# crowsonkb/style_transfer

Measured on AMD Instinct MI355X. Metric: tile-iterations/sec, VGG-19 2048px/1024-tile (fwd+bwd, Gram/content losses, regularizers, Adam step), higher is better.
Workload: dtype f32 (fp16x2-split MFMA, fp32 accumulate)

## Files before the change

include/stx.h:

```cpp
#ifndef STX_H_
#define STX_H_

#include <stddef.h>
#include <stdint.h>

#ifdef __cplusplus
extern "C" {
#endif

typedef struct stx_engine stx_engine;

typedef enum stx_status {
    STX_OK = 0,
    STX_ERR_ARG = -1,
    STX_ERR_HIP = -2,
    STX_ERR_STATE = -3,
    STX_ERR_UNSUPPORTED = -4,
    STX_ERR_NOMEM = -5
} stx_status;

typedef enum stx_mem { STX_HOST = 0, STX_DEVICE = 1 } stx_mem;

typedef enum stx_layer_type {
    STX_LAYER_INPUT = 0, STX_LAYER_CONV = 1, STX_LAYER_RELU = 2, STX_LAYER_POOL = 3
} stx_layer_type;

typedef enum stx_pool_mode { STX_POOL_MAX = 0, STX_POOL_AVE = 1 } stx_pool_mode;

typedef struct stx_layer_desc {
    const char *name;
    int type;
    const char *bottom;
    const char *top;
    int num_output;
    int kernel_size;
    int pad;
    int stride;
    int pool_mode;
} stx_layer_desc;

const char *stx_version(void);
const char *stx_last_error(void);
int stx_reread_env(void);
int stx_device_count(int *count);
int stx_device_name(int device, char *buf, size_t buf_len);

int stx_engine_create(int device, const stx_layer_desc *layers, int n_layers, stx_engine **out);
int stx_engine_create_shared(stx_engine *primary, stx_engine **out);
void stx_engine_destroy(stx_engine *e);
int stx_set_conv_weights(stx_engine *e, const char *conv_layer, const float *weights,
                         const float *bias, int mem);
int stx_sync(stx_engine *e);
int stx_fence(stx_engine *e, unsigned long long *ticket);
int stx_fence_wait(stx_engine *e, unsigned long long ticket);
int stx_engine_wait(stx_engine *e, stx_engine *other);
typedef enum stx_query {
    STX_Q_SHARED_ENGINES = 0,
    STX_Q_TARGET_UPLOADS = 1,
    STX_Q_TARGET_BYTES = 2,
    STX_Q_WEIGHT_BYTES = 3,
    STX_Q_TILE_EVALS = 4,
    STX_Q_PEERS_WITHOUT_ACCESS = 5
} stx_query;
int stx_engine_query(stx_engine *e, int what, double *value);
int stx_engine_device(stx_engine *e, int *device);
int stx_engine_stream(stx_engine *e, void **hip_stream);

int stx_malloc(stx_engine *e, size_t bytes, void **dev_ptr);
int stx_free(stx_engine *e, void *dev_ptr);
int stx_memset_async(stx_engine *e, void *dev_ptr, int value, size_t bytes);
int stx_memcpy_async(stx_engine *e, void *dst, int dst_mem, const void *src, int src_mem,
                     size_t bytes);

typedef struct stx_content_target {
    int content_index;
    const char *layer;
    int channels, height, width;
    const float *features;
    int mem;
} stx_content_target;

typedef struct stx_style_target {
    int style_index;
    const char *layer;
    int channels;
    const float *gram;
    int mem;
} stx_style_target;

int stx_set_contents_and_styles(stx_engine *e, const stx_content_target *contents, int n_contents,
                                const stx_style_target *styles, int n_styles);

typedef struct stx_style_mask {
    int style_index;
    int H, W;
    const float *mask;
    int mem;
} stx_style_mask;
int stx_set_style_masks(stx_engine *e, const stx_style_mask *masks, int n);

typedef struct stx_stat_target {
    const char *layer;
    int channels;
    const float *mean;
    const float *sd;
    int mem;
    double weight;
} stx_stat_target;
int stx_set_stat_targets(stx_engine *e, const stx_stat_target *targets, int n);

int stx_features_tile(stx_engine *e, const float *img, int img_mem, int th, int tw,
                      const char *const *layers, int n_layers, float *const *out, int out_mem);

typedef struct stx_tap {
    const char *layer;
    double layer_weight;
    int is_content;
    double content_weight;
    int is_style;
    double style_weight;
    int is_dd;
    double dd_weight;
} stx_tap;

int stx_sc_grad_tile(stx_engine *e, const float *img, int img_mem, int th, int tw,
                     const int roll_xy[2], const int start_yx[2], const stx_tap *taps, int n_taps,
                     double *loss_out, float *grad_out, int grad_mem, int sync_now);

int stx_tile_buffers(stx_engine *e, int th, int tw, float **tile_in, float **grad_out);

int stx_gram_matrix(stx_engine *e, const float *feat, int feat_mem, int channels, int hw,
                    float *gram_out, int gram_mem);

int stx_feature_stats(stx_engine *e, const float *feat, int feat_mem, int channels, int hw,
                      float *mean_out, float *sd_out, int out_mem);


int stx_image_cut_tile(stx_engine *e, const float *img, int H, int W, const int roll_xy[2],
                       int y0, int x0, int th, int tw, float *tile);
int stx_image_put_tile(stx_engine *e, float *grad, int H, int W, const int roll_xy[2],
                       int y0, int x0, int th, int tw, const float *tile_grad);

int stx_image_mask_map(stx_engine *e, const float *mask, int H, int W, int scale, float *out);
int stx_map_place(stx_engine *e, float *dst, int channels, int dst_h, int dst_w, int y0, int x0,
                  const float *src, int h, int w);
int stx_map_roll_add(stx_engine *e, float *acc, const float *src, int channels, int h, int w,
                     const int roll_xy[2], double alpha, double init_divisor);

int stx_image_resample(stx_engine *e, const float *src, int channels, int H, int W, float *dst,
                       int out_h, int out_w, const int *bounds_x, const double *weights_x,
                       int ksize_x, const int *bounds_y, const double *weights_y, int ksize_y,
                       int clamp_min_zero);

int stx_image_regularizers(stx_engine *e, const float *img, float *grad, int H, int W,
                           const float mean_bgr[3], double tv_scale, double tv_power,
                           double p_scale, double p_power, const float *aux, double aux_scale,
                           const int aux_roll_xy[2], double *loss_out);

int stx_image_swt_haar(stx_engine *e, const float *img, float *grad, int H, int W,
                       const int roll_xy[2], double scale, double power, double *loss_out);

int stx_image_swt_haar_levels(stx_engine *e, const float *img, float *grad, int H, int W, int levels,
                              const int roll_xy[2], double scale, double power, double *loss_out);

int stx_image_swt_daub_levels(stx_engine *e, const float *img, float *grad, int H, int W,
                              int order, int levels, const int *roll_xy,
                              double scale, double power, double *loss_out);

int stx_adam_step(stx_engine *e, float *params, const float *grad, float *g1, float *g2, float *p1,
                  float *avg_out, size_t n, double lr, double b1, double b2, double bp1,
                  double corr1, double corr2, double corrp);

int stx_vec_dot(stx_engine *e, const float *x, const float *y, size_t n, double *out_host_sync);
int stx_vec_axpy(stx_engine *e, double a, const float *x, float *y, size_t n);
int stx_vec_scale(stx_engine *e, double a, float *x, size_t n);
int stx_vec_mean_abs(stx_engine *e, const float *x, size_t n, double *out_host_sync);
int stx_vec_dot_async(stx_engine *e, const float *x, const float *y, size_t n, double *out_dev);
int stx_vec_abs_sum_async(stx_engine *e, const float *x, size_t n, double *out_dev);
int stx_vec_axpy_dev(stx_engine *e, double c1, const double *a_dev, double da, double c2,
                     const double *b_dev, double db, const float *x, float *y, size_t n);
int stx_vec_scale_dev(stx_engine *e, double c, const double *den_dev, double den_div, float *x,
                      size_t n);
int stx_vec_axpy_dot_dev(stx_engine *e, double c1, const double *a_dev, double da, double c2,
                         const double *b_dev, double db, double scale_c, const double *scale_den_dev,
                         double scale_div, const float *x, const float *src, float *y, const float *z,
                         size_t n, double *out_dev);
int stx_vec_lbfgs_pair(stx_engine *e, const float *g_new, float *g_old, const float *s, float *y, size_t n,
                       double *out_dev2, double *sy_host_sync);
int stx_vec_scale2_axpy(stx_engine *e, double c1, double c2, float *s, float *params, size_t n);

int stx_image_step_stats(stx_engine *e, const float *avg, float *old, int H, int W,
                         double stats[2]);
int stx_image_step_stats_async(stx_engine *e, const float *avg, float *old, int H, int W,
                               double raw_sums[2]);

int stx_image_to_u8(stx_engine *e, const float *img, int H, int W, const float mean_bgr[3],
                    uint8_t *out_rgb_u8);

int stx_image_to_u8_luma(stx_engine *e, const float *img, const float *content, int H, int W,
                         const float mean_bgr[3], uint8_t *out_rgb_u8);
int stx_image_color_stats(stx_engine *e, const float *img, int H, int W, double out_host_sync[9]);
int stx_image_color_affine(stx_engine *e, const float *src, float *dst, int H, int W, const double A[9],
                           const double b[3], const float mean_bgr[3]);

size_t stx_image_lap_floats(int H, int W, int n_pools, const int *pools);
int stx_image_lap_target(stx_engine *e, const float *content, int H, int W, int n_pools,
                         const int *pools, float *target_out);
int stx_image_lap(stx_engine *e, const float *img, float *grad, int H, int W, int n_pools,
                  const int *pools, const double *weights, const float *target, double scale,
                  double *loss_out);

int stx_op_conv_forward(stx_engine *e, const float *x, int Cin, int H, int W, const float *w,
                        const float *b, int Cout, int ksize, int relu, float *y);
int stx_op_conv_backward_data(stx_engine *e, const float *dy, int Cout, int H, int W,
                              const float *w, int Cin, int ksize, const float *relu_mask_data,
                              float *dx);
int stx_op_pool_forward(stx_engine *e, const float *x, int C, int H, int W, int mode, float *y);
int stx_op_pool_backward(stx_engine *e, const float *dy, const float *x, int C, int H, int W,
                         int mode, const float *relu_mask_data, float *dx);

int stx_op_style_terms(stx_engine *e, const float *feat, int channels, int h, int w,
                       const float *gram_target, float *s_out, float *normalized_out,
                       double *half_sumsq, double *abs_sum);
int stx_op_masked_style_terms(stx_engine *e, const float *feat, int channels, int h, int w,
                              const float *mask_map, int mh, int mw, int oy, int ox, const int roll_xy[2],
                              const float *gram_target, float *sgrad_out, double out[3]);
int stx_op_stat_terms(stx_engine *e, const float *feat, int channels, int h, int w, const float *MU,
                      const float *SD, float *s_out, double out[2]);
int stx_op_content_terms(stx_engine *e, const float *feat, int channels, int h, int w,
                         const float *content, int content_h, int content_w, int oy, int ox,
                         const int roll_xy[2], float *normalized_out, double sums[2]);

int stx_profile_enable(stx_engine *e, int on);
int stx_profile_read(stx_engine *e, char *buf, size_t buf_len, size_t *needed);

int stx_last_tile_ms(stx_engine *e, float *ms);

int stx_last_tile_flops(stx_engine *e, double *algorithmic, double *issued);

int stx_clock_marks(stx_engine *e, int on);
int stx_clock_marks_read(stx_engine *e, double *mhz, int max_values, int *n_values);

#ifdef __cplusplus
}
#endif
#endif
```

style_transfer_amd/csrc/common.h:

```cpp
#pragma once

#include <hip/hip_runtime.h>

#include <vector>

#include <cstdarg>
#include <cstdio>
#include <functional>
#include <string>

#include "stx.h"

namespace stx {

constexpr float kEps = 1.1920928955078125e-07f;

void set_error(const char *fmt, ...);

const char *sw_env(const char *name);
void sw_reread();

#define STX_HIP(call)                                                                       \
    do {                                                                                    \
        hipError_t err__ = (call);                                                          \
// ... 40 lines not shown
#pragma unroll
    for (int k = 0; k < NV; ++k) {
        const float s = wave_sum_f(v[k]);
        if ((threadIdx.x & 63) == 0) red[k][threadIdx.x >> 6] = s;
    }
    __syncthreads();
    if (threadIdx.x == 0) {
#pragma unroll
        for (int k = 0; k < NV; ++k)
            partials[k * gridDim.x + blockIdx.x] = red[k][0] + red[k][1] + red[k][2] + red[k][3];
    }
}

__device__ __forceinline__ unsigned pool_max_code(float v00, float v01, float v10, float v11, bool hx,
                                                  bool hy) {
    unsigned arg = 0;
    float best = v00;
    if (hx && v01 > best) best = v01, arg = 1;
    if (hy && v10 > best) best = v10, arg = 2;
    if (hx && hy && v11 > best) best = v11, arg = 3;
    return arg | (best > 0.f ? 4u : 0u);
}
__device__ __forceinline__ unsigned pool_ave_code(float v00, float v01, float v10, float v11, bool hx,
                                                  bool hy) {
    return (v00 > 0.f ? 1u : 0u) | (hx && v01 > 0.f ? 2u : 0u) | (hy && v10 > 0.f ? 4u : 0u) |
           (hx && hy && v11 > 0.f ? 8u : 0u);
}
#endif


enum ConvEpilogue {
    kEpiForward = 0,
    kEpiDgrad = 1,
    kEpiSymm = 2,
    kEpiDgradInject = 3,
    kEpiPartial = 4
};

struct ContentWindow {
    int C, fh, fw;
    int ch, cw;
    int oy, ox;
    int sy, sx;
};

struct ConvInject {
    const float *sgrad = nullptr, *s_abs_sum = nullptr;
    float s_coef = 0.f;
    const float *content = nullptr, *c_sums = nullptr, *feat = nullptr;
    float c_coef = 0.f;
    ContentWindow win{};
};

struct ConvProblem {
    const float *x;
    const float *w;
    float *y;
    const float *bias;
    const float *mask;
    float *partials;
    int K, M, H, W;
    int ksize;
    int relu;
    int epilogue;
    ConvInject inject;
    unsigned char *pool_codes = nullptr;
    unsigned char *in_codes = nullptr;
    const unsigned char *mask_codes = nullptr;
    unsigned char *out_codes = nullptr;
    bool wants_codes = false;
    bool skip_y = false;
    float *pool_out = nullptr;
    int pool_mode = 0;
    float *splitk_ws = nullptr;
    size_t splitk_ws_floats = 0;
    long long *clock_out = nullptr;
    const unsigned *x_amax = nullptr;
    unsigned *y_amax = nullptr;
    const unsigned char *pin_codes = nullptr;
    int pin_mode = 0;
    bool pin_mask = false;
#ifdef STX_EXPERIMENT_BF3
    const void *x_split = nullptr;
#endif
};

enum class ConvFamily { Direct, Wino2, H2 };

struct ConvConfig {
    ConvFamily family;
    int id;
    int bm;
    int kc;
    int pr, pc;
    int threads;
    size_t lds_bytes;
};

ConvConfig conv_pick_config(int ksize, int K, int M, int H, int W);
ConvConfig conv_config_by_id(int id);
bool direct_takes_inject(const ConvConfig &cfg);
int conv_num_workgroups(const ConvConfig &cfg, int M, int H, int W);
size_t conv_packed_floats(const ConvConfig &cfg, int K, int M, int ksize);
int conv_pack_weights(hipStream_t s, const float *w_caffe, int Mo, int Ko, int ksize,
                      int transpose_flip, const ConvConfig &cfg, float *packed);
int conv_launch(hipStream_t s, const ConvConfig &cfg, const ConvProblem &p, bool packed_weights);
int direct_splitk_factor(const ConvConfig &cfg, const ConvProblem &p, bool packed_weights);

int splitk_reduce_launch(hipStream_t s, const ConvProblem &p, int ksplit);
int splitk_reduce_items_launch(hipStream_t s, const ConvProblem &p, const ConvConfig &cfg, int slices,
                               int item_base, int items);
__host__ __device__ inline void wino2_item_tiles(int lt, int m_tiles, int n_patches, int &pt, int &mt) {
    pt = lt / m_tiles;
    mt = lt - pt * m_tiles;
    if (m_tiles == 8 && (n_patches & 7) == 0) {
        const int g = lt >> 5, r = lt & 31;
        mt = (g & 1) * 4 + (r & 3);
        pt = (g >> 1) * 8 + (r >> 2);
    }
}

struct WinoArgs {
    const float *x;
    const float *w;
    float *y;
    const float *bias;
    const float *mask;
    int K, M, H, W;
    int n_chunks, tiles_x, tiles_y, m_tiles, ksplit;
    int w_tile_stride;
    int x_bytes, w_bytes;
    int relu;
    ConvInject inj;
    float *pool_out;
    int pool_mode;
    unsigned char *pool_codes;
    int skip_y = 0;
    unsigned char *out_codes = nullptr;
    unsigned char *in_codes = nullptr;
    const unsigned char *mask_codes = nullptr;
    long long *clock_out = nullptr;
    int item_base = 0;
    const unsigned *x_amax = nullptr;
    unsigned *y_amax = nullptr;
    const unsigned char *pin_codes = nullptr;
    int pin_mode = 0, pin_mask = 0;
#ifdef STX_EXPERIMENT_BF3
    int vp_rows = 0, vp_tp = 0;
#endif
};

bool conv_first_usable(int K, int M, int ksize);
int conv_first_workgroups(int H, int W);
int conv_first_launch(hipStream_t s, const float *x, const float *w_caffe, const float *bias, float *y,
                      int K, int H, int W, int relu, float *gram_partials, unsigned *y_amax = nullptr);

ConvConfig wino2_config(int geometry = 0);
int wino2_pick_geometry(int H, int W);
size_t wino2_packed_floats(int K, int M);
int wino2_pack_weights(hipStream_t s, const float *w_caffe, int Mo, int Ko, int transpose_flip,
                       float *packed);
int wino2_launch(hipStream_t s, const ConvConfig &cfg, const ConvProblem &p, int ksplit);
bool wino2_fuses_pool(const ConvProblem &p);
bool wino2_uses_relu_codes(const ConvProblem &p, int ksplit);
bool wino2_writes_out_codes(const ConvConfig &cfg, const ConvProblem &p);
int wino2_splitk_factor(const ConvConfig &cfg, const ConvProblem &p);
struct Wino2Tail { int items, slices; };
Wino2Tail wino2_tail_split(const ConvConfig &cfg, const ConvProblem &p);
int wino2_max_slices(const ConvConfig &cfg, const ConvProblem &p);

constexpr int kAmaxSlots = 64;
ConvConfig h2_config(int mb, int pb = 1);
ConvConfig h2_pick_config(const ConvProblem &p);
bool h2_usable(const ConvProblem &p);
size_t h2_packed_floats(int K, int M);
int h2_pack_weights(hipStream_t s, const float *w_caffe, int Mo, int Ko, int transpose_flip, float *packed);
int h2_launch(hipStream_t s, const ConvConfig &cfg, const ConvProblem &p, int ksplit);
int h2_splitk_factor(const ConvConfig &cfg, const ConvProblem &p);
bool h2_fuses_pool(const ConvProblem &p);
bool h2_takes_pooled_input(const ConvConfig &cfg, const ConvProblem &p);
int absmax_launch(hipStream_t s, const float *x, size_t n, unsigned *slots);

size_t conv_small_packed_floats(int K);
int conv_small_pack(hipStream_t s, const float *w_caffe, int Mo, int Ko, int transpose_flip,
                    float *packed);
int conv_small_launch(hipStream_t s, const float *x, const float *packed, float *y,
                      const float *mask, int K, int M, int H, int W);

bool conv_h2_enabled();
struct ConvTuner { int device; hipStream_t stream; hipEvent_t ev0, ev1; std::function<int(const ConvConfig &, const float **)> bank; };
int conv_choose(const ConvProblem &p, bool winograd, const ConvTuner *tuner, ConvConfig *out);
struct ConvBank { int key; size_t floats; std::function<int(hipStream_t, const float *w_caffe, float *packed)> pack; };
ConvBank conv_bank(const ConvConfig &cfg, int dir, int Mo, int Ko, int ksize);
ConvBank conv_small_bank(int Mo, int Ko);
int conv_dispatch(hipStream_t s, const ConvConfig &cfg, const ConvProblem &p, double *flop_algorithmic,
                  double *flop_issued);
int conv_splitk_factor(const ConvConfig &cfg, const ConvProblem &p);
size_t conv_splitk_floats(const ConvConfig &cfg, const ConvProblem &p);
bool conv_takes_clock(const ConvConfig &cfg);
bool conv_fuses_pool(const ConvConfig &cfg, const ConvProblem &p);
bool conv_writes_pool_codes(const ConvConfig &cfg);
bool conv_reads_x_amax(const ConvConfig &cfg);
bool conv_leaves_y_amax(const ConvConfig &cfg);
bool conv_takes_inject(const ConvConfig &cfg);
bool conv_takes_pooled_input(const ConvConfig &cfg, const ConvProblem &p);
bool conv_uses_relu_codes(const ConvConfig &cfg, const ConvProblem &p, int ksplit);
bool conv_writes_out_codes(const ConvConfig &cfg, const ConvProblem &p, int ksplit);

int pool_forward_launch(hipStream_t s, const float *x, int C, int H, int W, int mode, float *y,
                        unsigned char *codes = nullptr);
int pool_backward_codes_launch(hipStream_t s, const float *dy, const unsigned char *codes, int C,
                               int H, int W, int mode, bool relu_mask, float *dx);
int pool_backward_launch(hipStream_t s, const float *dy, const float *x, int C, int H, int W,
                         int mode, bool relu_mask, float *dx);

struct GramPlan {
    int C, HW, splits, tiles;
    int parts;
    size_t partial_floats;
};
GramPlan gram_plan(int C, int HW);
bool gram_h2_usable(const float *feat, int C, int HW);
int gram_partials_launch(hipStream_t s, const float *feat, const GramPlan &plan, float *partials,
                         const unsigned *f_amax = nullptr);
int gram_finish_blocks(const GramPlan &plan);
int gram_finish_launch(hipStream_t s, const float *partials, const GramPlan &plan, float *gram_out,
                       const float *target, float *dsym, float *sumsq, unsigned short *pieces = nullptr,
                       const unsigned *f_amax = nullptr, float *block_out = nullptr);

size_t symm_pieces_elems(int C);
int symm_num_workgroups(int C, int HW);
bool symm_bf3_usable(const float *feat, const float *out, int C, int HW);
bool symm_h2_usable(const float *feat, const float *out, int C, int HW);
int symm_h2_launch(hipStream_t s, const float *feat, const float *dsym, const unsigned *d_amax, int n_damax,
                   const unsigned *f_amax, float *out, float *partials, int C, int HW);
int symm_bf3_launch(hipStream_t s, const float *feat, const float *dsym, unsigned short *pieces,
                    bool pieces_ready, float *out, float *partials, int C, int HW);

#ifdef __HIPCC__
__device__ __forceinline__ int content_origin_y(const ContentWindow &w) { return w.oy - w.sy; }
__device__ __forceinline__ int content_origin_x(const ContentWindow &w) { return w.ox - w.sx; }
__device__ __forceinline__ size_t content_index(const ContentWindow &w, int c, int y, int x) {
    int yy = (content_origin_y(w) + y) % w.ch;
    int xx = (content_origin_x(w) + x) % w.cw;
    if (yy < 0) yy += w.ch;
    if (xx < 0) xx += w.cw;
    return ((size_t)c * w.ch + yy) * w.cw + xx;
}
#endif

struct SumJob {
    const float *src;
    int n;
    float *dst;
};
int sum_jobs_launch(hipStream_t s, const SumJob *jobs, int n_jobs);
int content_sums_launch(hipStream_t s, const float *feat, const float *content,
                        const ContentWindow &win, float *sums , std::vector<SumJob> *defer = nullptr);
int inject_style_launch(hipStream_t s, float *diff, const float *sgrad, size_t n,
                        const float *abs_sum, float coef, bool accumulate, unsigned *y_amax = nullptr);
int inject_content_launch(hipStream_t s, float *diff, const float *feat, const float *content,
                          const ContentWindow &win, const float *sums, float coef, bool accumulate,
                          unsigned *y_amax = nullptr);
int relu_inplace_launch(hipStream_t s, float *x, size_t n);
int sum_partials_launch(hipStream_t s, const float *partials, int n, float *out);
int sum_partials2_launch(hipStream_t s, const float *a, int na, float *out_a, const float *b, int nb,
                         float *out_b);

constexpr int kMaskParts = 1024;
constexpr int kMaskSgradParts = 2048;
int mask_map_launch(hipStream_t s, const float *mask, int H, int W, int scale, float *out);
int mask_apply_launch(hipStream_t s, const float *feat, const float *map, const ContentWindow &win, float *fm,
                      float *m2_partials, int *n_parts);
int mask_target_launch(hipStream_t s, const float *gs, int C, const float *m2_partials, int n_parts, int HW,
                       float *out, float *a_out);
int mask_sgrad_launch(hipStream_t s, float *sgrad, const float *map, const ContentWindow &win, const float *a,
                      float *partials, int *n_parts);

constexpr int kStatSlice = 16384;
constexpr float kStatEps = 1e-5f;
int stat_slices(int HW);
size_t stat_scratch_floats(int C, int HW);
int stat_partials_launch(hipStream_t s, const float *feat, int C, int HW, float *partials);
int stat_finish_launch(hipStream_t s, const float *partials, int C, int HW, const float *MU, const float *SD,
                       float *table, float *e_out, float *mean_out, float *sd_out);
int stat_grad_launch(hipStream_t s, const float *feat, int C, int HW, const float *table, float *sgrad,
                     float *abs_partials, int *n_parts);

int cut_tile_launch(hipStream_t s, const float *img, int H, int W, int rx, int ry, int y0, int x0,
                    int th, int tw, float *tile);
int put_tile_launch(hipStream_t s, float *grad, int H, int W, int rx, int ry, int y0, int x0,
                    int th, int tw, const float *tile);
int place_window_launch(hipStream_t s, float *dst, int dh, int dw, int y0, int x0, const float *src,
                        int C, int h, int w);
int roll_add_launch(hipStream_t s, float *acc, const float *src, int C, int h, int w, int sx, int sy,
                    float alpha, bool init);
int resample_launch(hipStream_t s, int axis, const float *src, int C, int H, int W, float *dst,
                    int OH, int OW, const int *bounds, const double *k, int ksize, int clamp);
int finish_partials_launch(hipStream_t s, const float *partials, int n, double *out_dev);
int finish_partials_n_launch(hipStream_t s, const float *partials, int n, int nv, double *out_dev);
int regularizers_launch(hipStream_t s, const float *img, float *grad, int H, int W,
                        const float mean[3], float tv_scale, float tv_power, float p_scale,
                        float p_power, const float *aux, float aux_scale, int aux_rx, int aux_ry,
                        double *loss_terms , float *scratch, size_t scratch_floats);

int swt_padded_side(int H, int W);
int swt_haar_launch(hipStream_t s, const float *img, float *grad, int H, int W, int rx, int ry,
                    float scale, float power, double *loss_term, float *scratch,
                    size_t scratch_floats);
void swt_levels_scratch(int H, int W, size_t *tmp_floats, size_t *partial_floats);
int swt_haar_levels_launch(hipStream_t s, const float *img, float *grad, int H, int W, int levels,
                           int rx, int ry, float scale, float power, double *loss_term, float *tmp,
                           float *partials);
void swt_daub_table(int order, int levels, int N, std::vector<float> *taps, int *hl);
int swt_table_launch(hipStream_t s, const float *img, float *grad, int H, int W, const float *table,
                     int ntaps, int hl, int rx, int ry, float scale, float power,
                     double *loss_term, float *tmp, float *partials);

constexpr int kLapMaxPools = 4;
struct LapLevels {
    int n;
    int lp[kLapMaxPools], hp[kLapMaxPools], wp[kLapMaxPools], off[kLapMaxPools];
};
size_t lap_levels(int H, int W, int n_pools, const int *pools, LapLevels *lv);
size_t lap_scratch_floats(size_t map_floats);
int lap_target_launch(hipStream_t s, const float *content, int H, int W, const LapLevels &lv,
                      float *target, float *scratch);
int lap_launch(hipStream_t s, const float *img, float *grad, int H, int W, const LapLevels &lv,
               size_t map_floats, const float *coefs, const float *target, double *loss_terms,
               float *scratch);

int adam_launch(hipStream_t s, float *params, const float *grad, float *g1, float *g2, float *p1,
                float *avg, size_t n, double lr, double b1, double b2, double bp1, double c1,
                double c2, double cp);
int dot_launch(hipStream_t s, const float *x, const float *y, size_t n, double *out_dev,
               float *scratch, size_t scratch_floats);
int abs_sum_launch(hipStream_t s, const float *x, size_t n, double *out_dev, float *scratch,
                   size_t scratch_floats);
int axpy_launch(hipStream_t s, float a, const float *x, float *y, size_t n);
int scale_launch(hipStream_t s, float a, float *x, size_t n);
// ... 22 lines not shown
```

style_transfer_amd/csrc/conv_first.hip:

```cpp

#include <algorithm>
#include <cstdlib>

#include "bf16x3.h"
#include "common.h"

namespace stx {

namespace {

constexpr int kFP = 128;
constexpr int kFM = 64;
constexpr int kPW = kFP + 4;
constexpr int kPatch = 12 * kPW;
constexpr int kFLd = kFP + 4;
constexpr int kTile = kFM * kFLd;
constexpr int kNT = 256;
constexpr int kPL = (9 * (kFP + 2) + kNT - 1) / kNT;

typedef float f32x16 __attribute__((ext_vector_type(16)));
typedef float f32x4 __attribute__((ext_vector_type(4)));
typedef unsigned int u32x4f __attribute__((ext_vector_type(4)));

__device__ __forceinline__ int sgpr(int v) { return __builtin_amdgcn_readfirstlane(v); }
__device__ __forceinline__ void lds_barrier() { asm volatile("s_waitcnt lgkmcnt(0)\n\ts_barrier" ::: "memory"); }

struct FirstArgs {
    const float *x;
    const float *w;
    const float *bias;
    float *y;
    float *gram;
    unsigned *y_amax;
    int K, H, W, tiles_x, n_tiles, relu, vec_store, strided;
};

}

template <bool GRAM, int STORE>
__global__ __launch_bounds__(kNT, GRAM ? 2 : 3) void conv_first_kernel(FirstArgs a) {
    constexpr int kWork = 2 * kPatch + kTile;
    static_assert(kFM * kFM <= kWork, "the Gram tile must fit the working set");
    __shared__ __attribute__((aligned(16))) float lds[kWork];
    float *const patch = lds;
    float *const tile = lds + 2 * kPatch;
    const int tid = threadIdx.x, lane = tid & 63;
    const int wave = __builtin_amdgcn_readfirstlane(tid >> 6);
    const int l31 = lane & 31, half = lane >> 5;
    const size_t HW = (size_t)a.H * a.W;

    float aw[2][18];
#pragma unroll
    for (int s = 0; s < 18; ++s) {
        const int c = 2 * (s / 9) + half, tap = s % 9;
#pragma unroll
        for (int mb = 0; mb < 2; ++mb)
            aw[mb][s] = c < a.K ? a.w[((size_t)(mb * 32 + l31) * a.K + c) * 9 + tap] : 0.f;
    }
#pragma unroll
    for (int s = 0; s < 18; ++s) asm volatile("" ::"v"(aw[0][s]), "v"(aw[1][s]));
    float bias_r[2];
#pragma unroll
    for (int mb = 0; mb < 2; ++mb) bias_r[mb] = a.bias ? a.bias[mb * 32 + l31] : 0.f;
    asm volatile("" ::"v"(bias_r[0]), "v"(bias_r[1]));

    const __amdgpu_buffer_rsrc_t rx = __builtin_amdgcn_make_buffer_rsrc(
        const_cast<float *>(a.x), 0, (int)((size_t)a.K * HW * 4), 0x00020000);
    constexpr unsigned kOob = 0x80000000u;
    int p_row[kPL], p_col[kPL], p_off[kPL];
#pragma unroll
    for (int n = 0; n < kPL; ++n) {
        const int e = tid + n * kNT;
        const int pr = e / (kFP + 2), col = e - pr * (kFP + 2);
        const int c = pr / 3, r = pr - 3 * c;
        const bool live = e < 9 * (kFP + 2) && c < a.K;
        p_row[n] = live ? r - 1 : -(1 << 28);
        p_col[n] = col - 1;
        p_off[n] = (c * a.H + r - 1) * a.W + col - 1;
    }
    auto patch_load = [&](int t, float (&preg)[kPL]) {
        const int ty = sgpr(t < 0 ? -4 : t / a.tiles_x);
        const int x0 = sgpr(t < 0 ? 0 : (t - ty * a.tiles_x) * kFP);
        const int origin = sgpr(ty * a.W + x0);
#pragma unroll
        for (int n = 0; n < kPL; ++n) {
            const bool ok = (unsigned)(ty + p_row[n]) < (unsigned)a.H && (unsigned)(x0 + p_col[n]) < (unsigned)a.W;
            const unsigned off = ok ? (unsigned)(origin + p_off[n]) * 4u : kOob;
            preg[n] = __builtin_bit_cast(float, __builtin_amdgcn_raw_buffer_load_b32(rx, off, 0, 0));
        }
    };
    int p_dst[kPL];
#pragma unroll
    for (int n = 0; n < kPL; ++n) {
        const int e = tid + n * kNT;
        const int pr = e / (kFP + 2), col = e - pr * (kFP + 2);
        p_dst[n] = e < 9 * (kFP + 2) ? pr * kPW + col : -1;
    }
    auto patch_store = [&](int buf, const float (&preg)[kPL]) {
#pragma unroll
        for (int n = 0; n < kPL; ++n)
            if (p_dst[n] >= 0) patch[buf * kPatch + p_dst[n]] = preg[n];
    };

    f32x16 g[3];
    if (GRAM) {
#pragma unroll
        for (int b = 0; b < 3; ++b)
#pragma unroll
            for (int r = 0; r < 16; ++r) g[b][r] = 0.f;
    }

    const int per_wg = a.strided ? 1 : (a.n_tiles + (int)gridDim.x - 1) / (int)gridDim.x;
    const int grid = a.strided ? (int)gridDim.x : 1;
    const int t_begin = a.strided ? (int)blockIdx.x : (int)blockIdx.x * per_wg;
    const int t_end = a.strided ? a.n_tiles : (t_begin + per_wg < a.n_tiles ? t_begin + per_wg : a.n_tiles);
    const __amdgpu_buffer_rsrc_t ry = __builtin_amdgcn_make_buffer_rsrc(
        a.y, 0, STORE == 2 ? 0 : (int)(unsigned)((size_t)kFM * HW * 4), 0x00020000);
    constexpr unsigned kOobY = 0xfffffff0u;
    const int y_ch0 = tid >> 5, y_c4 = (tid & 31) * 4;
    const unsigned y_voff = (unsigned)(((size_t)y_ch0 * HW + y_c4) * 4);
    const bool track = a.y_amax != nullptr;
    float amax = 0.f;
    auto segment = [&](int t, int buf, const float (&pin)[kPL], float (&pout)[kPL]) {
        patch_load(t + 2 * grid < t_end ? t + 2 * grid : -1, pout);
        const int ty = sgpr(t / a.tiles_x), x0 = sgpr((t - ty * a.tiles_x) * kFP);

        f32x16 acc[2];
#pragma unroll
        for (int mb = 0; mb < 2; ++mb)
#pragma unroll
            for (int r = 0; r < 16; ++r) acc[mb][r] = 0.f;
        const float *pb = patch + buf * kPatch + half * (3 * kPW) + wave * 32 + l31;
#pragma unroll
        for (int s = 0; s < 18; ++s) {
            const int q = s / 9, ky = (s % 9) / 3, kx = s % 3;
            const float xv = pb[(2 * q * 3 + ky) * kPW + kx];
            acc[0] = __builtin_amdgcn_mfma_f32_32x32x2f32(xv, aw[0][s], acc[0], 0, 0, 0);
            acc[1] = __builtin_amdgcn_mfma_f32_32x32x2f32(xv, aw[1][s], acc[1], 0, 0, 0);
        }
        const bool ragged = x0 + kFP > a.W;
        const int room = a.W - x0 - wave * 32 - 4 * half;
#pragma unroll
        for (int mb = 0; mb < 2; ++mb)
#pragma unroll
            for (int j = 0; j < 4; ++j) {
                f32x4 v = {acc[mb][4 * j], acc[mb][4 * j + 1], acc[mb][4 * j + 2], acc[mb][4 * j + 3]};
                v += bias_r[mb];
                if (a.relu) {
                    v.x = fmaxf(v.x, 0.f), v.y = fmaxf(v.y, 0.f);
                    v.z = fmaxf(v.z, 0.f), v.w = fmaxf(v.w, 0.f);
                }
                if (ragged) {
                    v.x = 8 * j + 0 < room ? v.x : 0.f, v.y = 8 * j + 1 < room ? v.y : 0.f;
                    v.z = 8 * j + 2 < room ? v.z : 0.f, v.w = 8 * j + 3 < room ? v.w : 0.f;
                }
                if (track) amax = fmaxf(fmaxf(amax, fmaxf(fabsf(v.x), fabsf(v.y))), fmaxf(fabsf(v.z), fabsf(v.w)));
                *reinterpret_cast<f32x4 *>(tile + (mb * 32 + l31) * kFLd + wave * 32 + 8 * j + 4 * half) = v;
            }
        lds_barrier();

        {
            float *const yrow = a.y + (size_t)ty * a.W + x0;
            const unsigned origin = (unsigned)sgpr((ty * a.W + x0) * 4);
            const unsigned vo4 = x0 + y_c4 < a.W ? y_voff : kOobY;
#pragma unroll
            for (int n = 0; n < kFM * (kFP / 4) / kNT; ++n) {
                const f32x4 v = *reinterpret_cast<const f32x4 *>(tile + (y_ch0 + 8 * n) * kFLd + y_c4);
                if (STORE == 2) {
                    float *const dst = yrow + (size_t)(y_ch0 + 8 * n) * HW + y_c4;
                    if (x0 + y_c4 + 0 < a.W) dst[0] = v.x;
                    if (x0 + y_c4 + 1 < a.W) dst[1] = v.y;
                    if (x0 + y_c4 + 2 < a.W) dst[2] = v.z;
                    if (x0 + y_c4 + 3 < a.W) dst[3] = v.w;
                    continue;
                }
                const unsigned so = origin + (unsigned)sgpr((int)((unsigned)(8 * n) * (unsigned)HW * 4u));
                if (STORE == 0) {
                    __builtin_amdgcn_raw_buffer_store_b128(__builtin_bit_cast(u32x4f, v), ry, vo4, so, 0);
                } else {
                    const float vs[4] = {v.x, v.y, v.z, v.w};
#pragma unroll
                    for (int i = 0; i < 4; ++i)
                        __builtin_amdgcn_raw_buffer_store_b32(__builtin_bit_cast(unsigned, vs[i]), ry,
                                                              x0 + y_c4 + i < a.W ? y_voff + 4u * i : kOobY, so, 0);
                }
            }
        }
        if (GRAM) {
#pragma unroll
            for (int st = 0; st < 2; ++st) {
                bf16x8 p[2][3];
#pragma unroll
                for (int mb = 0; mb < 2; ++mb) {
                    const float *q = tile + (mb * 32 + l31) * kFLd + wave * 32 + st * 16 + half * 8;
                    const f32x4 lo = *reinterpret_cast<const f32x4 *>(q);
                    const f32x4 hi = *reinterpret_cast<const f32x4 *>(q + 4);
                    const float xv[8] = {lo.x, lo.y, lo.z, lo.w, hi.x, hi.y, hi.z, hi.w};
                    split3_bf16(xv, p[mb][0], p[mb][1], p[mb][2]);
                }
                g[0] = mfma_split6(p[0], p[0], g[0]);
                g[1] = mfma_split6(p[1], p[0], g[1]);
                g[2] = mfma_split6(p[1], p[1], g[2]);
            }
        }
        if (t + grid < t_end) patch_store(buf ^ 1, pin);
        lds_barrier();
    };

    for (int i = tid; i < 2 * kPatch; i += kNT) patch[i] = 0.f;
    lds_barrier();
    float pa[kPL], pb2[kPL];
    const int t0 = t_begin;
    if (t0 < t_end) {
        patch_load(t0, pa);
        patch_store(0, pa);
    }
    if (t0 + grid < t_end) patch_load(t0 + grid, pa);
    lds_barrier();
    for (int t = t0; t < t_end; t += 2 * grid) {
        segment(t, 0, pa, pb2);
        if (t + grid < t_end) segment(t + grid, 1, pb2, pa);
    }

    if (track) {
#pragma unroll
        for (int d = 32; d >= 1; d >>= 1) amax = fmaxf(amax, __shfl_xor(amax, d));
        lds_barrier();
        if (lane == 0) lds[wave] = amax;
        lds_barrier();
        if (tid == 0)
            atomicMax(a.y_amax + (blockIdx.x & (kAmaxSlots - 1)),
                      __builtin_bit_cast(unsigned, fmaxf(fmaxf(lds[0], lds[1]), fmaxf(lds[2], lds[3]))));
    }
    if (GRAM) {
        lds_barrier();
        float *const red = lds;
#pragma unroll 1
        for (int w = 0; w < 4; ++w) {
            if (wave == w) {
#pragma unroll
                for (int r = 0; r < 16; ++r) {
                    const int row = (r & 3) + 8 * (r >> 2) + 4 * half;
                    float *q0 = red + row * kFM + l31, *q1 = red + (32 + row) * kFM + l31;
                    q0[0] = w == 0 ? g[0][r] : q0[0] + g[0][r];
                    if (w == 0) q0[32] = 0.f;
                    q1[0] = w == 0 ? g[1][r] : q1[0] + g[1][r];
                    q1[32] = w == 0 ? g[2][r] : q1[32] + g[2][r];
                }
            }
            lds_barrier();
        }
        float *out = a.gram + (size_t)blockIdx.x * (kFM * kFM);
#pragma unroll
        for (int n = 0; n < 4; ++n) {
            const int e = tid + kNT * n;
            reinterpret_cast<float4 *>(out)[e] = reinterpret_cast<const float4 *>(red)[e];
        }
    }
}

bool conv_first_usable(int K, int M, int ksize) {
    const char *env = sw_env("STX_CONV_FIRST_FUSED");
    if (env && atoi(env) == 0) return false;
    return ksize == 3 && K >= 1 && K <= 3 && M == kFM;
}

int conv_first_workgroups(int H, int W) {
    const long tiles = (long)H * ceil_div(W, kFP);
    return (int)std::min<long>(tiles, 512);
}
static int conv_first_plain_workgroups(int H, int W) {
    const long tiles = (long)H * ceil_div(W, kFP);
    const char *env = sw_env("STX_FIRST_WGS");
    return (int)std::min<long>(tiles, env ? atoi(env) : 768);
}

int conv_first_launch(hipStream_t s, const float *x, const float *w_caffe, const float *bias, float *y,
                      int K, int H, int W, int relu, float *gram_partials, unsigned *y_amax) {
    if (4.0 * K * (double)H * W >= 2147483648.0) {
        set_error("conv_first_launch: a %d x %d plane is beyond the buffer-addressing limit", H, W);
        return STX_ERR_UNSUPPORTED;
    }
    FirstArgs a;
    a.x = x;
    a.w = w_caffe;
    a.bias = bias;
    a.y = y;
    a.gram = gram_partials;
    a.y_amax = y_amax;
    a.K = K;
    a.H = H;
    a.W = W;
    a.tiles_x = ceil_div(W, kFP);
    a.n_tiles = H * a.tiles_x;
    a.relu = relu;
    a.vec_store = W % 4 == 0 && (reinterpret_cast<uintptr_t>(y) & 15) == 0;
    const int grid = gram_partials ? conv_first_workgroups(H, W) : conv_first_plain_workgroups(H, W);
    {
        const char *env = sw_env("STX_FIRST_STRIDED");
        a.strided = env && atoi(env) != 0;
    }
    const int store = 4.0 * kFM * (double)H * W >= 4294967280.0 ? 2 : a.vec_store ? 0 : 1;
#define STX_FIRST(G, S) conv_first_kernel<G, S><<<grid, kNT, 0, s>>>(a)
    if (gram_partials) {
        if (store == 0) STX_FIRST(true, 0);
        else if (store == 1) STX_FIRST(true, 1);
        else STX_FIRST(true, 2);
    } else {
        if (store == 0) STX_FIRST(false, 0);
        else if (store == 1) STX_FIRST(false, 1);
        else STX_FIRST(false, 2);
    }
#undef STX_FIRST
    STX_CHECK_LAUNCH();
    return STX_OK;
}

}
```

style_transfer_amd/csrc/conv_mfma.hip:

```cpp

#include <algorithm>
#include <cstdlib>

#include "common.h"

namespace stx {

typedef float f32x16 __attribute__((ext_vector_type(16)));
typedef unsigned int u32x4 __attribute__((ext_vector_type(4)));

struct ConvKernelArgs {
    const float *x;
    const float *w;
    float *y;
    const float *bias;
    const float *mask;
    float *partials;
    int K, M, H, W;
    int n_chunks;
    int tiles_x, tiles_y;
    int m_tiles;
    int ksplit;
    int w_row_stride;
    int w_tile_stride;
// ... 522 lines not shown
    if (p.epilogue == kEpiForward && packed) return launch_variant<ID, kEpiForward, true>(s, cfg, a, n_wg);
    if constexpr (v.inject) {
        if (inject && packed) return launch_variant<ID, kEpiDgradInject, true>(s, cfg, a, n_wg);
    }
    if (p.epilogue == kEpiDgrad && packed && !inject) return launch_variant<ID, kEpiDgrad, true>(s, cfg, a, n_wg);
    set_error("conv_launch: no kernel for config %d epilogue %d packed %d", cfg.id, p.epilogue, (int)packed);
    return STX_ERR_UNSUPPORTED;
}

int conv_launch(hipStream_t s, const ConvConfig &cfg, const ConvProblem &p, bool packed) {
    const ConvVariant &v = kVariants[cfg.id];
    if (v.ks != p.ksize) {
        set_error("conv_launch: config %d is %dx%d, problem is %dx%d", cfg.id, v.ks, v.ks, p.ksize,
                  p.ksize);
        return STX_ERR_ARG;
    }
    ConvKernelArgs a;
    a.x = p.x;
    a.w = p.w;
    a.y = p.y;
    a.bias = p.bias;
    a.mask = p.mask;
    a.partials = p.partials;
    a.K = p.K;
    a.M = p.M;
    a.H = p.H;
    a.W = p.W;
    a.n_chunks = ceil_div(p.K, cfg.kc);
    a.tiles_x = ceil_div(p.W, cfg.pc);
    a.tiles_y = ceil_div(p.H, cfg.pr);
    a.m_tiles = ceil_div(p.M, cfg.bm);
    a.w_row_stride = packed ? cfg.bm : p.M;
    a.w_tile_stride = packed ? a.n_chunks * cfg.kc * p.ksize * p.ksize * cfg.bm : 0;
    const double xb = 4.0 * p.K * (double)p.H * p.W;
    const double wb = packed ? 4.0 * (double)conv_packed_floats(cfg, p.K, p.M, p.ksize)
                             : 4.0 * (double)p.K * p.M;
    if (xb >= 2147483648.0 || wb >= 2147483648.0) {
        set_error("conv_launch: a %d x %d x %d plane set exceeds the 2 GiB buffer-addressing limit "
                  "of the kernel (use a smaller --tile-size)", p.K, p.H, p.W);
        return STX_ERR_UNSUPPORTED;
    }
    a.x_bytes = (int)xb;
    a.w_bytes = (int)wb;
    a.relu = p.relu;
    a.inj = p.inject;
    a.ksplit = 1;
    const bool inject = p.epilogue == kEpiDgrad && (p.inject.sgrad || p.inject.content);
    int n_wg = conv_num_workgroups(cfg, p.M, p.H, p.W);
    const int ksplit = direct_splitk_factor(cfg, p, packed);
    const bool split = ksplit > 1 && p.splitk_ws &&
                       p.splitk_ws_floats >= (size_t)ksplit * p.M * p.H * p.W;
    if (split) {
        a.ksplit = ksplit;
        a.y = p.splitk_ws;
        n_wg *= ksplit;
    }

    switch (cfg.id) {
#define STX_DISPATCH(ID) \
    case ID: return dispatch_variant<ID>(s, cfg, p, a, n_wg, packed, inject, split ? ksplit : 1);
        STX_DISPATCH(0)
        STX_DISPATCH(1)
        STX_DISPATCH(2)
        STX_DISPATCH(3)
        STX_DISPATCH(4)
        STX_DISPATCH(8)
        STX_DISPATCH(9)
        STX_DISPATCH(10)
        STX_DISPATCH(11)
        STX_DISPATCH(5)
        STX_DISPATCH(6)
        STX_DISPATCH(7)
        STX_DISPATCH(12)
        STX_DISPATCH(13)
        STX_DISPATCH(14)
#undef STX_DISPATCH
    }
    set_error("conv_launch: no kernel for config %d epilogue %d packed %d", cfg.id, p.epilogue, (int)packed);
    return STX_ERR_UNSUPPORTED;
}

static SplitReduceArgs splitk_reduce_args(const ConvProblem &p, int ksplit) {
    SplitReduceArgs r;
    r.part = p.splitk_ws;
    r.y = p.y;
    r.bias = p.bias;
    r.mask = p.mask;
    r.inj = p.inject;
    r.ksplit = ksplit;
    r.M = p.M;
    r.HW = p.H * p.W;
    r.W = p.W;
    r.relu = p.relu;
    r.epilogue = p.epilogue;
    r.y_amax = p.y_amax;
    return r;
}

int splitk_reduce_launch(hipStream_t s, const ConvProblem &p, int ksplit) {
    const SplitReduceArgs r = splitk_reduce_args(p, ksplit);
    const size_t n = (size_t)p.M * p.H * p.W;
    if (n >= ((size_t)1 << 32)) {
        set_error("splitk_reduce: %zu elements", n);
        return STX_ERR_UNSUPPORTED;
    }
    const uintptr_t ptrs = reinterpret_cast<uintptr_t>(r.part) | reinterpret_cast<uintptr_t>(r.y) |
                           reinterpret_cast<uintptr_t>(r.mask) | reinterpret_cast<uintptr_t>(r.inj.feat) |
                           reinterpret_cast<uintptr_t>(r.inj.sgrad);
    const char *env = sw_env("STX_REDUCE_VEC");
    if ((p.H * p.W) % 4 == 0 && (ptrs & 15) == 0 && n < (1u << 31) && !(env && atoi(env) == 0)) {
        const size_t n4 = n / 4;
        splitk_reduce_vec4_kernel<<<(int)std::min<size_t>((n4 + 255) / 256, p.y_amax ? 1024 : 4096), 256, 0, s>>>(r);
        STX_CHECK_LAUNCH();
        return STX_OK;
    }
    splitk_reduce_kernel<<<(int)std::min<size_t>((n + 255) / 256, p.y_amax ? 1024 : 4096), 256, 0, s>>>(r);
    STX_CHECK_LAUNCH();
    return STX_OK;
}

int splitk_reduce_items_launch(hipStream_t s, const ConvProblem &p, const ConvConfig &cfg, int slices,
                               int item_base, int items) {
    const SplitReduceArgs r = splitk_reduce_args(p, slices);
    if ((size_t)p.M * p.H * p.W >= ((size_t)1 << 32)) {
        set_error("splitk_reduce: %zu elements", (size_t)p.M * p.H * p.W);
        return STX_ERR_UNSUPPORTED;
    }
    ItemRange range;
    range.item_base = item_base;
    range.m_tiles = ceil_div(p.M, 64);
    range.tiles_x = ceil_div(p.W, cfg.pc);
    range.tiles_y = ceil_div(p.H, cfg.pr);
    range.pr = cfg.pr;
    range.pc = cfg.pc;
    range.H = p.H;
    splitk_reduce_items_kernel<<<items * kItemBlocks, 256, 0, s>>>(r, range);
    STX_CHECK_LAUNCH();
    return STX_OK;
}

}

namespace stx {

typedef float f32x4 __attribute__((ext_vector_type(4)));

struct SmallConvArgs {
    const float *x;
    const float *w;
    float *y;
    const float *mask;
    int K, M, H, W, n_chunks, tiles_x, x_bytes, w_bytes;
    int n_wg, wg_per_xcd;
};

template <int KC, int PR, bool VEC>
__global__ __launch_bounds__(256) void conv3x3_m4_kernel(SmallConvArgs a) {
    constexpr int PC = 64, XR = PR + 2, XC = VEC ? PC + 8 : PC + 2, X0 = VEC ? 3 : 0, NT = 256, RW = PR / 4;
    constexpr int X_FLOATS = KC * XR * XC, W_FLOATS = KC * 9 * 4;
    constexpr int NX = (KC * XR * (PC + 2) + NT - 1) / NT;
    constexpr int NV = KC * XR * (PC / 4);
    constexpr int NVT = (NV + NT - 1) / NT;
    constexpr int NH = KC * XR * 2;
    static_assert(W_FLOATS / 4 <= NT, "one float4 of weights per thread");
    constexpr int NHT = (NH + NT - 1) / NT;
    __shared__ __attribute__((aligned(16))) float Xl[X_FLOATS];
    __shared__ __attribute__((aligned(16))) float Wl[W_FLOATS];
    const int tid = threadIdx.x, lane = tid & 63;
    const int wave = __builtin_amdgcn_readfirstlane(tid >> 6);
    const int patch = sgpr((int)(blockIdx.x & 7) * a.wg_per_xcd + (int)(blockIdx.x >> 3));
    if (patch >= a.n_wg) return;
    const int y0 = sgpr((patch / a.tiles_x) * PR), x0 = sgpr((patch % a.tiles_x) * PC);
    const int HW = a.H * a.W;
    constexpr unsigned kOob = 0x80000000u;
    const bool big = a.x_bytes == 0;
    __amdgpu_buffer_rsrc_t rx = __builtin_amdgcn_make_buffer_rsrc(
        const_cast<float *>(a.x), 0, a.x_bytes, 0x00020000);
    const __amdgpu_buffer_rsrc_t rw = __builtin_amdgcn_make_buffer_rsrc(
        const_cast<float *>(a.w), 0, a.w_bytes, 0x00020000);
    unsigned xvoff[VEC ? 1 : NX], vvoff[VEC ? NVT : 1], hvoff[NHT];
    int vdst[VEC ? NVT : 1], hdst[NHT];
    if (VEC) {
#pragma unroll
        for (int n = 0; n < NVT; ++n) {
            const int e = tid + n * NT;
            const int ci = e / (XR * (PC / 4)), rem = e - ci * (XR * (PC / 4));
            const int r = rem / (PC / 4), c4 = rem - r * (PC / 4);
            const int yy = y0 - 1 + r, xx = x0 + 4 * c4;
            const bool ok = e < NV && (unsigned)yy < (unsigned)a.H && xx < a.W;
            vvoff[n] = ok ? (unsigned)(ci * HW + yy * a.W + xx) * 4u : kOob;
            vdst[n] = e < NV ? (ci * XR + r) * XC + X0 + 1 + 4 * c4 : -1;
        }
#pragma unroll
        for (int n = 0; n < NHT; ++n) {
            const int e = tid + n * NT;
            const int ci = e / (XR * 2), rem = e - ci * (XR * 2);
            const int r = rem >> 1, side = rem & 1;
            const int yy = y0 - 1 + r, xx = side ? x0 + PC : x0 - 1;
            const bool ok = e < NH && (unsigned)yy < (unsigned)a.H && (unsigned)xx < (unsigned)a.W;
            hvoff[n] = ok ? (unsigned)(ci * HW + yy * a.W + xx) * 4u : kOob;
            hdst[n] = e < NH ? (ci * XR + r) * XC + X0 + (side ? PC + 1 : 0) : -1;
        }
    } else {
#pragma unroll
        for (int n = 0; n < NX; ++n) {
            const int e = tid + n * NT;
            const int ci = e / (XR * XC), rem = e - ci * (XR * XC);
            const int r = rem / XC, c = rem - r * XC;
            const int yy = y0 - 1 + r, xx = x0 - 1 + c;
            const bool ok = e < X_FLOATS && (unsigned)yy < (unsigned)a.H && (unsigned)xx < (unsigned)a.W;
            xvoff[n] = ok ? (unsigned)(ci * HW + yy * a.W + xx) * 4u : kOob;
        }
    }
    const unsigned wvoff = tid < W_FLOATS / 4 ? (unsigned)tid * 16u : kOob;
    unsigned xreg[VEC ? 1 : NX], hreg[NHT];
    u32x4 vreg[VEC ? NVT : 1];
    u32x4 wreg;
    auto load_stage = [&](int chunk) {
        wreg = __builtin_amdgcn_raw_buffer_load_b128(rw, wvoff, (unsigned)chunk * (W_FLOATS * 4u), 0);
        unsigned xs = (unsigned)sgpr((int)((unsigned)chunk * (unsigned)(KC * HW) * 4u));
        if (big) {
            const int k0 = sgpr(chunk * KC);
            const int nk = a.K - k0 < KC ? a.K - k0 : KC;
            rx = __builtin_amdgcn_make_buffer_rsrc(const_cast<float *>(a.x) + (size_t)k0 * (size_t)HW, 0,
                                                   (nk > 0 ? nk : 0) * HW * 4, 0x00020000);
            xs = 0;
        }
        if (VEC) {
#pragma unroll
            for (int n = 0; n < NVT; ++n) vreg[n] = __builtin_amdgcn_raw_buffer_load_b128(rx, vvoff[n], xs, 0);
#pragma unroll
            for (int n = 0; n < NHT; ++n) hreg[n] = __builtin_amdgcn_raw_buffer_load_b32(rx, hvoff[n], xs, 0);
        } else {
#pragma unroll
            for (int n = 0; n < NX; ++n) xreg[n] = __builtin_amdgcn_raw_buffer_load_b32(rx, xvoff[n], xs, 0);
        }
    };
    auto store_stage = [&]() {
        if (tid < W_FLOATS / 4) reinterpret_cast<u32x4 *>(Wl)[tid] = wreg;
        if (VEC) {
#pragma unroll
            for (int n = 0; n < NVT; ++n)
                if (vdst[n] >= 0) *reinterpret_cast<u32x4 *>(Xl + vdst[n]) = vreg[n];
#pragma unroll
            for (int n = 0; n < NHT; ++n)
                if (hdst[n] >= 0) reinterpret_cast<unsigned *>(Xl)[hdst[n]] = hreg[n];
        } else {
#pragma unroll
            for (int n = 0; n < NX; ++n) {
                const int e = tid + n * NT;
                if (e < X_FLOATS) reinterpret_cast<unsigned *>(Xl)[e] = xreg[n];
            }
        }
    };
    f32x4 acc[RW];
#pragma unroll
    for (int r = 0; r < RW; ++r) acc[r] = f32x4{0.f, 0.f, 0.f, 0.f};
    const float *wl = Wl + (lane & 3);
    const float *xl = Xl + (wave * RW) * XC + X0 + lane;

    load_stage(0);
    store_stage();
    __syncthreads();
    for (int chunk = 0; chunk < a.n_chunks; ++chunk) {
        const bool more = chunk + 1 < a.n_chunks;
        if (more) load_stage(chunk + 1);
#pragma unroll
        for (int ci = 0; ci < KC; ++ci) {
#pragma unroll
            for (int t = 0; t < 9; ++t) {
                const float av = wl[(ci * 9 + t) * 4];
#pragma unroll
                for (int r = 0; r < RW; ++r) {
                    const float bv = xl[ci * (XR * XC) + (r + t / 3) * XC + t % 3];
                    acc[r] = __builtin_amdgcn_mfma_f32_4x4x1f32(av, bv, acc[r], 0, 0, 0);
                }
            }
        }
        __syncthreads();
        if (more) {
            store_stage();
            __syncthreads();
        }
    }
    const int xx = x0 + lane;
#pragma unroll
    for (int r = 0; r < RW; ++r) {
        const int yy = y0 + wave * RW + r;
        if (yy < a.H && xx < a.W) {
#pragma unroll
            for (int m = 0; m < 4; ++m) {
                if (m < a.M) {
                    const size_t idx = (size_t)m * HW + (size_t)yy * a.W + xx;
                    float v = acc[r][m];
                    if (a.mask) v = a.mask[idx] > 0.f ? v : 0.f;
                    a.y[idx] = v;
                }
            }
        }
    }
}

constexpr int kSmallKC = 4, kSmallPR = 16;

size_t conv_small_packed_floats(int K) { return (size_t)ceil_div(K, kSmallKC) * kSmallKC * 9 * 4; }

__global__ void pack_small_kernel(const float *__restrict__ w, int Mo, int Ko, int transpose_flip,
                                  int M, int K, int kpad, float *__restrict__ packed) {
    const int total = kpad * 9 * 4;
    for (int i = blockIdx.x * blockDim.x + threadIdx.x; i < total; i += gridDim.x * blockDim.x) {
        const int m = i & 3, t = (i >> 2) % 9, k = i / 36;
        float v = 0.f;
        if (m < M && k < K)
            v = transpose_flip ? w[((size_t)k * Ko + m) * 9 + (8 - t)] : w[((size_t)m * Ko + k) * 9 + t];
        packed[i] = v;
    }
}

int conv_small_pack(hipStream_t s, const float *w_caffe, int Mo, int Ko, int transpose_flip,
                    float *packed) {
    const int M = transpose_flip ? Ko : Mo, K = transpose_flip ? Mo : Ko;
    const int kpad = ceil_div(K, kSmallKC) * kSmallKC;
    pack_small_kernel<<<ceil_div(kpad * 36, 256), 256, 0, s>>>(w_caffe, Mo, Ko, transpose_flip, M, K,
                                                               kpad, packed);
    STX_CHECK_LAUNCH();
    return STX_OK;
}

int conv_small_launch(hipStream_t s, const float *x, const float *packed, float *y,
                      const float *mask, int K, int M, int H, int W) {
    if (M > 4) {
        set_error("conv_small_launch: M = %d > 4", M);
        return STX_ERR_ARG;
    }
    const double xb = 4.0 * K * (double)H * W;
    const char *force_big = sw_env("STX_WINO_BIG");
    const bool big = xb >= 2147483648.0 || (force_big && atoi(force_big) == 1);
    if (4.0 * kSmallKC * (double)H * W >= 2147483648.0) {
        set_error("conv_small_launch: a %d x %d plane is beyond the buffer-addressing limit", H, W);
        return STX_ERR_UNSUPPORTED;
    }
    SmallConvArgs a;
    a.x = x;
    a.w = packed;
    a.y = y;
    a.mask = mask;
    a.K = K;
    a.M = M;
    a.H = H;
    a.W = W;
    a.n_chunks = ceil_div(K, kSmallKC);
    a.tiles_x = ceil_div(W, 64);
    a.x_bytes = big ? 0 : (int)xb;
    a.w_bytes = (int)(conv_small_packed_floats(K) * 4);
    const char *novec = sw_env("STX_SMALL_NOVEC");
    const bool vec = W % 4 == 0 && (reinterpret_cast<uintptr_t>(x) & 15) == 0 && !(novec && atoi(novec));
    const bool tall = (long)a.tiles_x * ceil_div(H, kSmallPR) >= 1024;
    int pr = tall ? kSmallPR : kSmallPR / 2;
#ifdef STX_SMALL_SWEEP
    if (const char *tune = sw_env("STX_SMALL_TUNE")) {
        const int kc = atoi(tune) / 100, prr = atoi(tune) % 100;
        a.n_chunks = ceil_div(K, kc);
        a.n_wg = a.tiles_x * ceil_div(H, prr);
        a.wg_per_xcd = ceil_div(a.n_wg, 8);
        const int g = a.wg_per_xcd * 8;
#define STX_SWEEP(KC_, PR_) if (kc == KC_ && prr == PR_) { conv3x3_m4_kernel<KC_, PR_, true><<<g, 256, 0, s>>>(a); STX_CHECK_LAUNCH(); return STX_OK; }
        STX_SWEEP(4, 8) STX_SWEEP(4, 16) STX_SWEEP(4, 32) STX_SWEEP(8, 8) STX_SWEEP(8, 16) STX_SWEEP(8, 32) STX_SWEEP(16, 8) STX_SWEEP(16, 16)
#undef STX_SWEEP
    }
#endif
    a.n_wg = a.tiles_x * ceil_div(H, pr);
    a.wg_per_xcd = ceil_div(a.n_wg, 8);
    const int grid = a.wg_per_xcd * 8;
    if (tall) {
        if (vec) conv3x3_m4_kernel<kSmallKC, kSmallPR, true><<<grid, 256, 0, s>>>(a);
        else conv3x3_m4_kernel<kSmallKC, kSmallPR, false><<<grid, 256, 0, s>>>(a);
    } else {
        if (vec) conv3x3_m4_kernel<kSmallKC, kSmallPR / 2, true><<<grid, 256, 0, s>>>(a);
        else conv3x3_m4_kernel<kSmallKC, kSmallPR / 2, false><<<grid, 256, 0, s>>>(a);
    }
    STX_CHECK_LAUNCH();
    return STX_OK;
}

}
```

style_transfer_amd/csrc/engine.cpp:

```cpp

#include <algorithm>
#include <atomic>
#include <cstdlib>
#include <cstring>

#include "engine.h"

namespace stx {

static thread_local std::string g_error;

void set_error(const char *fmt, ...) {
    char buf[1024];
    va_list ap;
    va_start(ap, fmt);
    vsnprintf(buf, sizeof buf, fmt, ap);
    va_end(ap);
    g_error = buf;
}

int alloc_scalars(stx_engine *e, size_t n, size_t *index) {
    stx_engine::ScalarArena &a = e->A();
    if (a.used + n > e->scalars_cap) {
        set_error("scalar arena exhausted (%zu + %zu > %zu)", a.used, n, e->scalars_cap);
        return STX_ERR_NOMEM;
    }
    *index = a.used;
    a.used += n;
    return STX_OK;
}

int alloc_dscalars(stx_engine *e, size_t n, size_t *index) {
    stx_engine::ScalarArena &a = e->A();
    if (a.dused + n > e->dscalars_cap - 4) {
        set_error("double-scalar arena exhausted; call stx_sync more often");
        return STX_ERR_NOMEM;
    }
    *index = a.dused;
    a.dused += n;
    return STX_OK;
}

int copy_in(stx_engine *e, void *dst, const void *src, int mem, size_t bytes) {
    if (mem == STX_HOST)
        STX_HIP(hipMemcpyAsync(dst, src, bytes, hipMemcpyHostToDevice, e->stream));
    else
        STX_HIP(hipMemcpyAsync(dst, src, bytes, hipMemcpyDefault, e->stream));
    return STX_OK;
}

int copy_out(stx_engine *e, void *dst, int mem, const void *src, size_t bytes) {
    if (mem == STX_HOST)
        STX_HIP(hipMemcpyAsync(dst, src, bytes, hipMemcpyDeviceToHost, e->stream));
    else
        STX_HIP(hipMemcpyAsync(dst, src, bytes, hipMemcpyDefault, e->stream));
    return STX_OK;
}

static void publish_arena(stx_engine::ScalarArena &a) {
    for (const PendingLoss &pl : a.pending) {
        double v = 0.0;
        for (const LossTerm &t : pl.terms) v += t.coef * (double)a.host[t.scalar_index];
        for (const LossTerm &t : pl.dterms) v += t.coef * a.dhost[t.scalar_index];
        if (pl.out) *pl.out = v;
    }
    a.pending.clear();
    a.used = 0;
    a.dused = 0;
    a.ticket = 0;
}

int do_sync(stx_engine *e) {
    STX_HIP(hipStreamSynchronize(e->stream));
    publish_arena(e->arena[e->cur ^ 1]);
    publish_arena(e->arena[e->cur]);
    return STX_OK;
}

static int quiesce_members(stx_engine *e) {
    for (stx_engine *m : e->sh->members) STX_HIP(hipStreamSynchronize(m->stream));
    return STX_OK;
}

namespace {
typedef std::map<std::string, std::string> SwitchMap;
std::atomic<const SwitchMap *> g_switches{nullptr};
std::mutex g_switches_mutex;
extern "C" char **environ;

const SwitchMap *switches_snapshot() {
    auto *m = new SwitchMap;
    for (char **e = environ; e && *e; ++e) {
        if (strncmp(*e, "STX_", 4) != 0) continue;
        const char *eq = strchr(*e, '=');
        if (eq) (*m)[std::string(*e, eq - *e)] = eq + 1;
    }
    return m;
}
}

void sw_reread() {
    std::lock_guard<std::mutex> lock(g_switches_mutex);
    g_switches.store(switches_snapshot(), std::memory_order_release);
}

const char *sw_env(const char *name) {
    const SwitchMap *m = g_switches.load(std::memory_order_acquire);
    if (!m) {
        std::lock_guard<std::mutex> lock(g_switches_mutex);
        m = g_switches.load(std::memory_order_acquire);
        if (!m) {
            m = switches_snapshot();
            g_switches.store(m, std::memory_order_release);
        }
    }
    auto it = m->find(name);
    return it == m->end() ? nullptr : it->second.c_str();
}
}

extern "C" {

const char *stx_version(void) { return "libstx 0.1 (gfx950)"; }

int stx_reread_env(void) {
    stx::sw_reread();
    return STX_OK;
}

const char *stx_last_error(void) { return g_error.c_str(); }

int stx_device_count(int *count) {
    if (!count) return STX_ERR_ARG;
    int n = 0;
    hipError_t err = hipGetDeviceCount(&n);
    if (err != hipSuccess) {
        (void)hipGetLastError();
        n = 0;
    }
    *count = n;
    return STX_OK;
}

int stx_device_name(int device, char *buf, size_t buf_len) {
    if (!buf || !buf_len) return STX_ERR_ARG;
    hipDeviceProp_t prop;
    STX_HIP(hipGetDeviceProperties(&prop, device));
    snprintf(buf, buf_len, "%s", prop.gcnArchName);
    return STX_OK;
}

}

static std::mutex g_peer_mutex;
static std::map<int, std::vector<int>> g_peers_missing;

void enable_peer_access(int device) {
    std::lock_guard<std::mutex> lock(g_peer_mutex);
    if (g_peers_missing.count(device)) return;
    std::vector<int> &missing = g_peers_missing[device];
    int n_dev = 0;
    if (hipGetDeviceCount(&n_dev) != hipSuccess) {
        (void)hipGetLastError();
        return;
    }
    for (int peer = 0; peer < n_dev; ++peer) {
        if (peer == device) continue;
        int can = 0;
        hipError_t err = hipDeviceCanAccessPeer(&can, device, peer);
        if (err == hipSuccess && can) {
            err = hipDeviceEnablePeerAccess(peer, 0);
            if (err == hipErrorPeerAccessAlreadyEnabled) err = hipSuccess;
        } else if (err == hipSuccess) {
            err = hipErrorPeerAccessUnsupported;
        }
        (void)hipGetLastError();
        if (err != hipSuccess) {
            missing.push_back(peer);
            fprintf(stderr, "libstx: no peer access GPU %d -> GPU %d (%s); copies between them are "
                            "staged by the runtime\n", device, peer, hipGetErrorString(err));
        }
    }
}

int peers_without_access(int device) {
    std::lock_guard<std::mutex> lock(g_peer_mutex);
    auto it = g_peers_missing.find(device);
    return it == g_peers_missing.end() ? 0 : (int)it->second.size();
}

constexpr size_t kScalarFloats = 1 << 18;

static int build_engine(int device, const stx_layer_desc *layers, int n_layers,
                        std::shared_ptr<SharedState> share, stx_engine **out) {
    if (!layers || n_layers < 2 || !out) {
        set_error("stx_engine_create: bad arguments");
        return STX_ERR_ARG;
    }
    if (layers[0].type != STX_LAYER_INPUT || !layers[0].top) {
        set_error("stx_engine_create: layer 0 must be the input layer");
        return STX_ERR_ARG;
    }
    std::unique_ptr<stx_engine> e(new stx_engine);
    e->device = device;
    const bool joined = share != nullptr;
    e->sh = joined ? share : std::make_shared<SharedState>();
    hipError_t err = hipSetDevice(device);
    if (err != hipSuccess) {
        set_error("hipSetDevice(%d): %s", device, hipGetErrorString(err));
        return STX_ERR_HIP;
    }
    auto add_blob = [&](const std::string &name, int channels, int producer) {
        Blob b;
        b.name = name;
        b.channels = channels;
        b.producer = producer;
        e->blob_index[name] = (int)e->blobs.size();
        e->blobs.push_back(std::move(b));
        return (int)e->blobs.size() - 1;
    };
    for (int i = 0; i < n_layers; ++i) {
        const stx_layer_desc &d = layers[i];
        Layer L;
        L.name = d.name ? d.name : "";
        L.bottom = d.bottom ? d.bottom : "";
// ... 77 lines not shown
        STX_HIP(hipEventCreate(&e->ev_stop[i]));
    }
    STX_HIP(hipEventCreate(&e->ev_tune0));
    STX_HIP(hipEventCreate(&e->ev_tune1));
    if (const char *env = sw_env("STX_AUTOTUNE")) e->autotune = atoi(env) != 0;
    if (const char *env = sw_env("STX_POOL_CODES")) e->pool_codes = atoi(env) != 0;
    if (const char *env = sw_env("STX_WINOGRAD")) e->winograd = atoi(env) != 0;
    e->scalars_cap = kScalarFloats;
    for (stx_engine::ScalarArena &a : e->arena) {
        STX_TRY(a.scalars.ensure(e->scalars_cap * sizeof(float)));
        STX_HIP(hipHostMalloc(reinterpret_cast<void **>(&a.host), e->scalars_cap * sizeof(float),
                              hipHostMallocDefault));
        STX_TRY(a.dscalars.ensure(e->dscalars_cap * sizeof(double)));
        STX_HIP(hipHostMalloc(reinterpret_cast<void **>(&a.dhost), e->dscalars_cap * sizeof(double),
                              hipHostMallocDefault));
        STX_HIP(hipEventCreateWithFlags(&a.fence, hipEventDisableTiming));
    }
    STX_TRY(e->red_scratch.ensure(9 * kBlocks * sizeof(float)));
    {
        std::lock_guard<std::mutex> lock(e->sh->mutex);
        e->sh->members.push_back(e.get());
    }
    *out = e.release();
    return STX_OK;
}

extern "C" {

int stx_engine_create(int device, const stx_layer_desc *layers, int n_layers, stx_engine **out) {
    return build_engine(device, layers, n_layers, nullptr, out);
}

int stx_engine_create_shared(stx_engine *primary, stx_engine **out) {
    if (!primary || !out) {
        set_error("stx_engine_create_shared: bad arguments");
        return STX_ERR_ARG;
    }
    std::vector<stx_layer_desc> descs(primary->layers.size());
    for (size_t i = 0; i < descs.size(); ++i) {
        const Layer &L = primary->layers[i];
        stx_layer_desc &d = descs[i];
        d.name = L.name.c_str();
        d.type = L.type;
        d.bottom = L.bottom.empty() ? nullptr : L.bottom.c_str();
        d.top = L.top.c_str();
        d.num_output = i == 0 ? primary->blobs[L.top_blob].channels : L.num_output;
        d.kernel_size = L.ksize;
        d.pad = L.pad;
        d.stride = L.stride;
        d.pool_mode = L.pool_mode;
    }
    STX_TRY(primary->set_device());
    for (stx_engine *m : primary->sh->members) STX_HIP(hipStreamSynchronize(m->stream));
    return build_engine(primary->device, descs.data(), (int)descs.size(), primary->sh, out);
}

void stx_engine_destroy(stx_engine *e) {
    if (!e) return;
    (void)hipSetDevice(e->device);
    if (e->stream) (void)hipStreamSynchronize(e->stream);
    for (auto &b : e->sgrad_tap) b->release();
    for (auto &b : e->sgrad_stat) b->release();
    e->marks_buf.release();
    e->amax.release();
    for (Blob &b : e->blobs) {
        b.data.release();
        b.diff.release();
        b.codes.release();
        b.relu_codes.release();
    }
    for (hipEvent_t ev : e->fence_events) (void)hipEventDestroy(ev);
    bool last;
    {
        std::lock_guard<std::mutex> lock(e->sh->mutex);
        auto &m = e->sh->members;
        m.erase(std::remove(m.begin(), m.end(), e), m.end());
        last = m.empty();
    }
    if (last) {
        for (auto &kv : e->sh->conv) {
            kv.second.w.release();
            kv.second.b.release();
            for (auto &p : kv.second.packed) p.second->release();
        }
        for (auto &c : e->sh->contents) c.feat->release();
        for (auto &s : e->sh->styles) s.gram->release();
        for (auto &m : e->sh->masks) m.map->release();
        for (auto &t : e->sh->stats) t.ms->release();
    }
    DevBuf *bufs[] = {&e->stat_scratch, &e->masked_feat, &e->masked_target, &e->splitk, &e->gram_partials, &e->gram, &e->dsym, &e->dsym_pieces, &e->symm_partials,
                      &e->upload, &e->red_scratch, &e->swt_scratch, &e->lap_scratch, &e->first_gram, &e->color_sums};
    for (DevBuf *b : bufs) b->release();
    for (stx_engine::SwtTable &t : e->swt_tables) t.taps.release();
    for (stx_engine::ScalarArena &a : e->arena) {
        a.scalars.release();
        a.dscalars.release();
        if (a.host) (void)hipHostFree(a.host);
        if (a.dhost) (void)hipHostFree(a.dhost);
        if (a.fence) (void)hipEventDestroy(a.fence);
    }
    for (auto &pe : e->prof) {
        (void)hipEventDestroy(pe.start);
        (void)hipEventDestroy(pe.stop);
    }
    for (hipEvent_t ev : e->event_pool) (void)hipEventDestroy(ev);
    for (int i = 0; i < stx_engine::kTimed; ++i) {
        if (e->ev_start[i]) (void)hipEventDestroy(e->ev_start[i]);
        if (e->ev_stop[i]) (void)hipEventDestroy(e->ev_stop[i]);
    }
    if (e->ev_tune0) (void)hipEventDestroy(e->ev_tune0);
    if (e->ev_tune1) (void)hipEventDestroy(e->ev_tune1);
    if (e->stream) (void)hipStreamDestroy(e->stream);
    delete e;
}

int stx_set_conv_weights(stx_engine *e, const char *conv_layer, const float *weights,
                         const float *bias, int mem) {
    if (!e || !conv_layer || !weights) return STX_ERR_ARG;
    STX_TRY(e->set_device());
    auto it = e->layer_index.find(conv_layer);
    if (it == e->layer_index.end() || e->layers[it->second].type != STX_LAYER_CONV) {
        set_error("stx_set_conv_weights: '%s' is not a convolution layer", conv_layer);
        return STX_ERR_ARG;
    }
    std::lock_guard<std::mutex> lock(e->sh->mutex);
    const bool shared = e->sh->members.size() > 1;
    if (shared) STX_TRY(quiesce_members(e));
    ConvParams &cp = e->sh->conv[it->second];
    const size_t nw = (size_t)cp.cout * cp.cin * cp.ks * cp.ks;
    STX_TRY(cp.w.ensure(nw * sizeof(float)));
    STX_TRY(cp.b.ensure((size_t)cp.cout * sizeof(float)));
    STX_TRY(copy_in(e, cp.w.ptr, weights, mem, nw * sizeof(float)));
    if (bias)
        STX_TRY(copy_in(e, cp.b.ptr, bias, mem, (size_t)cp.cout * sizeof(float)));
    else
        STX_HIP(hipMemsetAsync(cp.b.ptr, 0, (size_t)cp.cout * sizeof(float), e->stream));
    if (mem == STX_HOST || shared) STX_HIP(hipStreamSynchronize(e->stream));
    for (auto &p : cp.packed) p.second->release();
    cp.packed.clear();
    cp.set = true;
    return STX_OK;
}

int stx_sync(stx_engine *e) {
    if (!e) return STX_ERR_ARG;
    STX_TRY(e->set_device());
    return do_sync(e);
}

int stx_fence(stx_engine *e, unsigned long long *ticket) {
    if (!e || !ticket) return STX_ERR_ARG;
    STX_TRY(e->set_device());
    stx_engine::ScalarArena &a = e->A();
    STX_HIP(hipEventRecord(a.fence, e->stream));
    a.ticket = e->next_ticket++;
    *ticket = a.ticket;
    e->cur ^= 1;
    stx_engine::ScalarArena &b = e->A();
    if (b.ticket) {
        STX_HIP(hipEventSynchronize(b.fence));
        publish_arena(b);
    }
    return STX_OK;
}

int stx_fence_wait(stx_engine *e, unsigned long long ticket) {
    if (!e) return STX_ERR_ARG;
    STX_TRY(e->set_device());
    for (stx_engine::ScalarArena &a : e->arena) {
        if (a.ticket && a.ticket == ticket) {
            STX_HIP(hipEventSynchronize(a.fence));
            publish_arena(a);
        }
    }
    return STX_OK;
}

int stx_engine_device(stx_engine *e, int *device) {
    if (!e || !device) return STX_ERR_ARG;
    *device = e->device;
    return STX_OK;
}

int stx_engine_stream(stx_engine *e, void **hip_stream) {
    if (!e || !hip_stream) return STX_ERR_ARG;
    *hip_stream = e->stream;
    return STX_OK;
}

int stx_engine_wait(stx_engine *e, stx_engine *other) {
    if (!e || !other) return STX_ERR_ARG;
    if (e == other) return STX_OK;
    constexpr size_t kRing = 16;
    STX_TRY(other->set_device());
    if (other->fence_events.size() < kRing) {
        hipEvent_t ev;
        STX_HIP(hipEventCreateWithFlags(&ev, hipEventDisableTiming));
        other->fence_events.push_back(ev);
        other->fence_next = other->fence_events.size() - 1;
    }
    hipEvent_t ev = other->fence_events[other->fence_next];
    other->fence_next = (other->fence_next + 1) % kRing;
    STX_HIP(hipEventRecord(ev, other->stream));
    STX_TRY(e->set_device());
    STX_HIP(hipStreamWaitEvent(e->stream, ev, 0));
    return STX_OK;
}

int stx_engine_query(stx_engine *e, int what, double *value) {
    if (!e || !value) return STX_ERR_ARG;
    std::lock_guard<std::mutex> lock(e->sh->mutex);
    switch (what) {
        case STX_Q_SHARED_ENGINES: *value = (double)e->sh->members.size(); break;
        case STX_Q_TARGET_UPLOADS: *value = (double)e->sh->target_uploads; break;
        case STX_Q_TARGET_BYTES: *value = e->sh->target_bytes; break;
        case STX_Q_WEIGHT_BYTES: {
            double b = 0;
            for (auto &kv : e->sh->conv) {
                b += (double)kv.second.w.bytes + (double)kv.second.b.bytes;
                for (auto &p : kv.second.packed) b += (double)p.second->bytes;
            }
            *value = b;
            break;
        }
        case STX_Q_TILE_EVALS: *value = (double)e->n_tile_evals; break;
        case STX_Q_PEERS_WITHOUT_ACCESS: *value = (double)peers_without_access(e->device); break;
        default:
            set_error("stx_engine_query: unknown item %d", what);
            return STX_ERR_ARG;
    }
    return STX_OK;
}

int stx_malloc(stx_engine *e, size_t bytes, void **dev_ptr) {
    if (!e || !dev_ptr) return STX_ERR_ARG;
    STX_TRY(e->set_device());
    hipError_t err = hipMalloc(dev_ptr, bytes ? bytes : 4);
    if (err != hipSuccess) {
        set_error("hipMalloc(%zu): %s", bytes, hipGetErrorString(err));
        return STX_ERR_NOMEM;
    }
    return STX_OK;
}

int stx_free(stx_engine *e, void *dev_ptr) {
    if (!e) return STX_ERR_ARG;
    STX_TRY(e->set_device());
    if (dev_ptr) STX_HIP(hipFree(dev_ptr));
    return STX_OK;
}

int stx_memset_async(stx_engine *e, void *dev_ptr, int value, size_t bytes) {
    if (!e || !dev_ptr) return STX_ERR_ARG;
    STX_TRY(e->set_device());
    STX_HIP(hipMemsetAsync(dev_ptr, value, bytes, e->stream));
    return STX_OK;
}

int stx_memcpy_async(stx_engine *e, void *dst, int dst_mem, const void *src, int src_mem,
                     size_t bytes) {
    if (!e || !dst || !src) return STX_ERR_ARG;
    STX_TRY(e->set_device());
    hipMemcpyKind kind = hipMemcpyDefault;
    if (dst_mem == STX_HOST && src_mem == STX_HOST) kind = hipMemcpyHostToHost;
    if (dst_mem == STX_HOST && src_mem == STX_DEVICE) kind = hipMemcpyDeviceToHost;
    if (dst_mem == STX_DEVICE && src_mem == STX_HOST) kind = hipMemcpyHostToDevice;
    STX_HIP(hipMemcpyAsync(dst, src, bytes, kind, e->stream));
    return STX_OK;
}

int stx_set_contents_and_styles(stx_engine *e, const stx_content_target *contents, int n_contents,
                                const stx_style_target *styles, int n_styles) {
    if (!e || (n_contents && !contents) || (n_styles && !styles)) return STX_ERR_ARG;
    STX_TRY(e->set_device());
    std::lock_guard<std::mutex> lock(e->sh->mutex);
    const bool shared = e->sh->members.size() > 1;
    STX_TRY(quiesce_members(e));
    double copied = 0;
    for (auto &c : e->sh->contents) c.feat->release();
    for (auto &s : e->sh->styles) s.gram->release();
    for (auto &m : e->sh->masks) m.map->release();
    for (auto &t : e->sh->stats) t.ms->release();
    e->sh->contents.clear();
    e->sh->styles.clear();
    e->sh->masks.clear();
    e->sh->stats.clear();
    e->sh->n_contents = e->sh->n_styles = 0;
    bool host_src = false;
    for (int i = 0; i < n_contents; ++i) {
        const stx_content_target &c = contents[i];
        const int blob = e->find_blob(c.layer);
        if (blob < 0 || !c.features || c.channels != e->blobs[blob].channels || c.height <= 0 ||
            c.width <= 0 || c.content_index < 0) {
            set_error("content target %d: bad layer '%s' or shape", i, c.layer ? c.layer : "(null)");
            return STX_ERR_ARG;
        }
        ContentTarget t;
        t.index = c.content_index;
        t.blob = blob;
        t.C = c.channels;
        t.h = c.height;
        t.w = c.width;
        t.feat.reset(new DevBuf);
        const size_t bytes = (size_t)t.C * t.h * t.w * sizeof(float);
        STX_TRY(t.feat->ensure(bytes));
        STX_TRY(copy_in(e, t.feat->ptr, c.features, c.mem, bytes));
// ... 233 lines not shown
```

style_transfer_amd/csrc/engine.h:

```cpp
#pragma once

#include <map>
#include <memory>
#include <mutex>
#include <string>
#include <vector>

#include "common.h"

namespace stx {

struct DevBuf {
    void *ptr = nullptr;
    size_t bytes = 0;
    int ensure(size_t need) {
        if (need <= bytes) return STX_OK;
        if (ptr) STX_HIP(hipFree(ptr));
        ptr = nullptr;
        bytes = 0;
        const size_t want = (need + 255) & ~(size_t)255;
        hipError_t err = hipMalloc(&ptr, want);
        if (err != hipSuccess) {
            set_error("hipMalloc(%zu bytes) failed: %s", want, hipGetErrorString(err));
            ptr = nullptr;
            return STX_ERR_NOMEM;
        }
        bytes = want;
        return STX_OK;
    }
    void release() {
        if (ptr) (void)hipFree(ptr);
        ptr = nullptr;
        bytes = 0;
    }
    float *f() const { return static_cast<float *>(ptr); }
};

struct Layer {
    std::string name, bottom, top;
    int type = 0, num_output = 0, ksize = 0, pad = 0, stride = 1, pool_mode = 0;
    int bottom_blob = -1, top_blob = -1;
};

struct Blob {
    std::string name;
    int channels = 0;
    int producer = -1;
    bool relu = false;
    int scale = 1;
    int h = 0, w = 0;
    DevBuf data, diff;
    DevBuf codes;
    bool codes_valid = false;
    DevBuf relu_codes;
    bool relu_codes_valid = false;
    bool relu_codes_wanted = false;
    int amax_data = -1, amax_diff = -1;
    size_t count() const { return (size_t)channels * h * w; }
};

struct ConvParams {
    int cin = 0, cout = 0, ks = 0;
    DevBuf w, b;
    bool set = false;
    std::map<int, std::unique_ptr<DevBuf>> packed;
};

struct ContentTarget {
    int index, blob, C, h, w;
    std::unique_ptr<DevBuf> feat;
};

struct StyleTarget {
    int index, blob, C;
    std::unique_ptr<DevBuf> gram;
};

struct StyleMask {
    int index, blob, h, w;
    std::unique_ptr<DevBuf> map;
};

struct StatTarget {
    int blob, C;
    double weight;
    std::unique_ptr<DevBuf> ms;
};

struct LossTerm {
    size_t scalar_index;
    double coef;
};

struct PendingLoss {
    double *out;
    std::vector<LossTerm> terms;
    std::vector<LossTerm> dterms;
};

struct SharedState {
    std::map<int, ConvParams> conv;
    std::vector<ContentTarget> contents;
    std::vector<StyleTarget> styles;
    std::vector<StyleMask> masks;
    std::vector<StatTarget> stats;
    int n_contents = 0, n_styles = 0;
    std::vector<stx_engine *> members;
    std::mutex mutex;
    size_t target_uploads = 0;
    double target_bytes = 0;
};

}

using namespace stx;

struct stx_engine {
    int device = 0;
    hipStream_t stream = nullptr;
    bool clock_marks = false;
    DevBuf marks_buf;
    int marks_used = 0, last_mark = -1;
    std::vector<std::unique_ptr<DevBuf>> sgrad_tap;
    std::vector<std::unique_ptr<DevBuf>> sgrad_stat;
    static constexpr int kTimed = 4;
    hipEvent_t ev_start[kTimed] = {}, ev_stop[kTimed] = {};
    int ev_cur = 0;
    int ev_recorded = 0;
    hipEvent_t ev_tune0 = nullptr, ev_tune1 = nullptr;
    bool timed = false;
    double flop_algorithmic = 0, flop_issued = 0;
    std::vector<Layer> layers;
    std::vector<Blob> blobs;
    std::map<std::string, int> blob_index, layer_index;
    std::shared_ptr<SharedState> sh;

    DevBuf splitk;
    DevBuf amax;
    unsigned *amax_slots(int blob, bool diff) const {
        return static_cast<unsigned *>(amax.ptr) + ((size_t)(diff ? blobs.size() : 0) + blob) * kAmaxSlots;
    }
    int amax_ensure() {
        return amax.ensure((2 * blobs.size() + 2) * kAmaxSlots * sizeof(unsigned));
    }
    DevBuf first_gram;
    int first_gram_blob = -1, first_gram_parts = 0;
    bool first_gram_valid = false;
    DevBuf gram_partials, gram, dsym, dsym_pieces, symm_partials, upload;
    DevBuf term_scratch;
    DevBuf masked_feat, masked_target;
    DevBuf stat_scratch;
    struct ScalarArena {
        DevBuf scalars;
        float *host = nullptr;
        size_t used = 0;
        DevBuf dscalars;
        double *dhost = nullptr;
        size_t dused = 0;
        std::vector<PendingLoss> pending;
        hipEvent_t fence = nullptr;
        unsigned long long ticket = 0;
    };
    ScalarArena arena[2];
    int cur = 0;
    unsigned long long next_ticket = 1;
    ScalarArena &A() { return arena[cur]; }
    size_t scalars_cap = 0;
    size_t n_tile_evals = 0;
    std::vector<hipEvent_t> fence_events;
    size_t fence_next = 0;
    size_t dscalars_cap = 64;
    DevBuf red_scratch;
    DevBuf color_sums;
    DevBuf swt_scratch;
    struct SwtTable {
        int order, levels, N, ntaps, hl;
        DevBuf taps;
    };
    std::vector<SwtTable> swt_tables;
    DevBuf lap_scratch;

    bool winograd = true;
    bool autotune = true;
    bool pool_codes = true;

    bool profiling = false;
    struct ProfEntry {
        std::string label;
        double flops;
        hipEvent_t start, stop;
        int mark = -1;
    };
    std::vector<ProfEntry> prof;
    std::vector<hipEvent_t> event_pool;

    int set_device() {
        STX_HIP(hipSetDevice(device));
        return STX_OK;
    }
    int find_blob(const char *name) const {
        if (!name) return -1;
        auto it = blob_index.find(name);
        return it == blob_index.end() ? -1 : it->second;
    }
};

namespace stx {
#pragma GCC visibility push(hidden)

struct ProfScope {
    stx_engine *e;
    int index = -1;
    hipStream_t stream;
    ProfScope(stx_engine *eng, const std::string &label, double flops, hipStream_t on = nullptr)
        : e(eng), stream(on ? on : eng->stream) {
        if (!e->profiling) return;
        auto take = [&]() {
            hipEvent_t ev = nullptr;
            if (!e->event_pool.empty()) {
                ev = e->event_pool.back();
                e->event_pool.pop_back();
            } else if (hipEventCreate(&ev) != hipSuccess) {
                ev = nullptr;
            }
            return ev;
        };
        stx_engine::ProfEntry pe{label, flops, take(), take()};
        if (!pe.start || !pe.stop) return;
        (void)hipEventRecord(pe.start, stream);
        e->prof.push_back(pe);
        index = (int)e->prof.size() - 1;
    }
    ~ProfScope() {
        if (index < 0) return;
        (void)hipEventRecord(e->prof[index].stop, stream);
        e->prof[index].mark = e->last_mark;
        e->last_mark = -1;
    }
};

constexpr int kMaxClockMarks = 16384;

int alloc_scalars(stx_engine *e, size_t n, size_t *index);
int alloc_dscalars(stx_engine *e, size_t n, size_t *index);
int copy_in(stx_engine *e, void *dst, const void *src, int mem, size_t bytes);
int copy_out(stx_engine *e, void *dst, int mem, const void *src, size_t bytes);
int do_sync(stx_engine *e);
ConvProblem conv_fwd_problem(const float *x, float *y, const float *bias, int Cin, int Cout, int H, int W,
                             int ks, int relu);
ConvProblem conv_bwd_problem(const float *dy, float *dx, const float *mask, int Cout, int Cin, int H, int W,
                             int ks);
int attach_splitk(stx_engine *e, const ConvConfig &cfg, ConvProblem &p);
int launch_conv(stx_engine *e, const ConvConfig &cfg, const ConvProblem &problem);
int amax_scratch(stx_engine *e, unsigned **out);
int launch_style_terms(stx_engine *e, hipStream_t stream, const float *feat, int C, int h, int w,
                       const float *target, float *sgrad, float *sc, const std::string &name,
                       const unsigned *f_amax = nullptr, float *term_scratch = nullptr,
                       std::vector<SumJob> *defer = nullptr);
constexpr size_t kMaskScratchFloats = kMaskParts + kMaskSgradParts;
int launch_masked_style_terms(stx_engine *e, hipStream_t stream, const float *feat, int C, int h, int w,
                              const float *mask_map, const ContentWindow &win, const float *target,
                              float *sgrad, float *sc, const std::string &name, const unsigned *f_amax,
                              float *term_scratch, float *mask_scratch, std::vector<SumJob> *defer);
int launch_stat_terms(stx_engine *e, hipStream_t stream, const float *feat, int C, int h, int w, const float *MU,
                      const float *SD, float *sgrad, float *sc, const std::string &name, float *stat_scratch,
                      std::vector<SumJob> *defer);
#pragma GCC visibility pop

}
```

style_transfer_amd/csrc/tile_path.cpp:

```cpp

#include <algorithm>
#include <cmath>
#include <cstdlib>
#include <deque>

#include "engine.h"

namespace stx {

ConvProblem conv_fwd_problem(const float *x, float *y, const float *bias, int Cin, int Cout, int H, int W,
                             int ks, int relu) {
    ConvProblem p{};
    p.x = x;
    p.y = y;
    p.bias = bias;
    p.K = Cin;
    p.M = Cout;
    p.H = H;
    p.W = W;
    p.ksize = ks;
    p.relu = relu;
    p.epilogue = kEpiForward;
    return p;
}

ConvProblem conv_bwd_problem(const float *dy, float *dx, const float *mask, int Cout, int Cin, int H, int W,
                             int ks) {
    ConvProblem p{};
    p.x = dy;
    p.y = dx;
    p.mask = mask;
    p.K = Cout;
    p.M = Cin;
    p.H = H;
    p.W = W;
    p.ksize = ks;
    p.epilogue = kEpiDgrad;
    return p;
}

static double conv_flops(int K, int M, int H, int W, int ks) {
    return 2.0 * K * M * ks * ks * (double)H * W;
}

static int shape_blobs(stx_engine *e, int th, int tw, const std::vector<char> &needed, bool with_diff) {
    Blob &in = e->blobs[e->layers[0].top_blob];
    in.h = th;
    in.w = tw;
    for (size_t li = 1; li < e->layers.size(); ++li) {
        const Layer &L = e->layers[li];
        if (L.type == STX_LAYER_RELU) continue;
        const Blob &b = e->blobs[L.bottom_blob];
        Blob &t = e->blobs[L.top_blob];
        if (L.type == STX_LAYER_CONV) {
            t.h = b.h;
            t.w = b.w;
        } else {
            t.h = pooled_len(b.h);
            t.w = pooled_len(b.w);
        }
    }
    for (size_t bi = 0; bi < e->blobs.size(); ++bi) {
        if (!needed[bi]) continue;
        Blob &b = e->blobs[bi];
        STX_TRY(b.data.ensure(b.count() * sizeof(float)));
        if (with_diff) STX_TRY(b.diff.ensure(b.count() * sizeof(float)));
    }
    return STX_OK;
}

static void mark_ancestors(const stx_engine *e, int blob, std::vector<char> &needed) {
    while (blob >= 0 && !needed[blob]) {
        needed[blob] = 1;
        const int p = e->blobs[blob].producer;
        if (p <= 0) break;
        blob = e->layers[p].bottom_blob;
    }
}

static int get_bank(stx_engine *e, int layer, const ConvBank &bank, const float **out) {
    std::lock_guard<std::mutex> lock(e->sh->mutex);
    ConvParams &cp = e->sh->conv[layer];
    if (!cp.set) {
        set_error("weights of layer %s were never set", e->layers[layer].name.c_str());
        return STX_ERR_STATE;
    }
    auto it = cp.packed.find(bank.key);
    if (it == cp.packed.end()) {
        std::unique_ptr<DevBuf> buf(new DevBuf);
        STX_TRY(buf->ensure(bank.floats * sizeof(float)));
        STX_TRY(bank.pack(e->stream, cp.w.f(), buf->f()));
        if (e->sh->members.size() > 1) STX_HIP(hipStreamSynchronize(e->stream));
        it = cp.packed.emplace(bank.key, std::move(buf)).first;
    }
    *out = it->second->f();
    return STX_OK;
}

static int get_packed(stx_engine *e, int layer, int dir, const ConvConfig &cfg, const float **out) {
    const ConvParams &cp = e->sh->conv[layer];
    return get_bank(e, layer, conv_bank(cfg, dir, cp.cout, cp.cin, cp.ks), out);
}

static int choose_conv(stx_engine *e, int li, int dir, const ConvProblem &p, ConvConfig *out) {
    const ConvTuner tuner{e->device, e->stream, e->ev_tune0, e->ev_tune1, [=](const ConvConfig &cfg, const float **w) {
                              return get_packed(e, li, dir, cfg, w);
                          }};
    return conv_choose(p, e->winograd, e->autotune ? &tuner : nullptr, out);
}

int attach_splitk(stx_engine *e, const ConvConfig &cfg, ConvProblem &p) {
    const size_t need = conv_splitk_floats(cfg, p);
    if (!need) return STX_OK;
    STX_TRY(e->splitk.ensure(need * sizeof(float)));
    p.splitk_ws = e->splitk.f();
    p.splitk_ws_floats = e->splitk.bytes / sizeof(float);
    return STX_OK;
}

int launch_conv(stx_engine *e, const ConvConfig &cfg, const ConvProblem &problem) {
    ConvProblem p = problem;
    e->last_mark = -1;
    if (e->clock_marks && conv_takes_clock(cfg) && e->marks_used < kMaxClockMarks) {
        e->last_mark = e->marks_used++;
        p.clock_out = static_cast<long long *>(e->marks_buf.ptr) + 2 * (size_t)e->last_mark;
    }
    return conv_dispatch(e->stream, cfg, p, &e->flop_algorithmic, &e->flop_issued);
}

static int amax_for(stx_engine *e, int blob, bool diff, const unsigned **out) {
    Blob &b = e->blobs[blob];
    int &src = diff ? b.amax_diff : b.amax_data;
    if (src < 0) {
        ProfScope scope(e, std::string("absmax ") + b.name, 0.0);
        STX_TRY(absmax_launch(e->stream, diff ? b.diff.f() : b.data.f(), b.count(), e->amax_slots(blob, diff)));
        src = blob;
    }
    *out = e->amax_slots(src, diff);
    return STX_OK;
}

int amax_scratch(stx_engine *e, unsigned **out) {
    STX_TRY(e->amax_ensure());
    *out = e->amax_slots((int)e->blobs.size(), true);
    return STX_OK;
}

struct FwdConvPlan {
    bool force_relu;
    const Layer *pool;
    int pool_li;
    bool top_unobserved;
    bool conv_reader;
    bool relu_codes;
};

static FwdConvPlan plan_fwd_conv(const stx_engine *e, size_t li, const std::vector<char> &needed, int relu_blob,
                                 bool relu_codes, const std::vector<char> &observed) {
    const Layer &L = e->layers[li];
    FwdConvPlan plan{L.top_blob == relu_blob, nullptr, -1, false, false, relu_codes};
    int readers = 0;
    for (size_t lj = li + 1; lj < e->layers.size(); ++lj) {
        const Layer &P = e->layers[lj];
        if (P.type == STX_LAYER_RELU || P.bottom_blob != L.top_blob) continue;
        ++readers;
        plan.conv_reader |= P.type == STX_LAYER_CONV && needed[P.top_blob];
        if (!plan.pool && P.type == STX_LAYER_POOL && needed[P.top_blob] && P.ksize == 2 && P.stride == 2 &&
            P.pad == 0 && !e->blobs[P.top_blob].relu && P.top_blob != relu_blob) {
            plan.pool = &P;
            plan.pool_li = (int)lj;
        }
    }
    plan.top_unobserved = plan.pool && !observed[L.top_blob] && L.top_blob != relu_blob && readers == 1;
    return plan;
}

static int run_conv_forward(stx_engine *e, int li, const FwdConvPlan &plan, bool *pooled) {
    const Layer &L = e->layers[li];
    const Layer *const pool = plan.pool;
    Blob &b = e->blobs[L.bottom_blob];
    Blob &t = e->blobs[L.top_blob];
    const ConvParams &cp = e->sh->conv[li];
    ConvProblem p = conv_fwd_problem(b.data.f(), t.data.f(), cp.b.f(), cp.cin, cp.cout, b.h, b.w, cp.ks,
                                     (t.relu || plan.force_relu) ? 1 : 0);
    const double direct = conv_flops(cp.cin, cp.cout, b.h, b.w, cp.ks);
    *pooled = false;
    if (conv_first_usable(cp.cin, cp.cout, cp.ks) && !pool) {
        b.relu_codes_valid = false;
        b.relu_codes_wanted = false;
        t.relu_codes_valid = false;
        unsigned *y_amax = nullptr;
        t.amax_data = -1;
        if (conv_h2_enabled()) {
            y_amax = e->amax_slots(L.top_blob, false);
            t.amax_data = L.top_blob;
        }
        float *gram = nullptr;
        if (L.top_blob == e->first_gram_blob) {
            const int parts = conv_first_workgroups(b.h, b.w);
            STX_TRY(e->first_gram.ensure(((size_t)parts * 64 * 64 + 64 * 64 / 64 + 64) * sizeof(float)));
            gram = e->first_gram.f();
            e->first_gram_parts = parts;
            e->first_gram_valid = true;
        }
        ProfScope scope(e, "fwd " + L.name, direct);
        e->flop_algorithmic += direct;
        e->flop_issued += direct;
        return conv_first_launch(e->stream, p.x, cp.w.f(), cp.b.f(), p.y, cp.cin, b.h, b.w, p.relu, gram, y_amax);
    }
    ConvConfig cfg;
    STX_TRY(choose_conv(e, li, 0, p, &cfg));
    b.relu_codes_wanted = !conv_reads_x_amax(cfg) && !b.relu_codes_valid && plan.relu_codes && b.relu && b.channels <= 128;
    p.wants_codes = b.relu_codes_wanted;
    t.amax_data = -1;
    if (conv_reads_x_amax(cfg)) STX_TRY(amax_for(e, L.bottom_blob, false, &p.x_amax));
    if (conv_leaves_y_amax(cfg)) {
        p.y_amax = e->amax_slots(L.top_blob, false);
        t.amax_data = L.top_blob;
    }
    STX_TRY(get_packed(e, li, 0, cfg, &p.w));
    STX_TRY(attach_splitk(e, cfg, p));
    if (b.relu_codes_wanted) {
        const size_t bytes = (size_t)b.channels * ((b.h + 1) / 2) * ((b.w + 1) / 2);
        STX_TRY(b.relu_codes.ensure(bytes));
        p.in_codes = static_cast<unsigned char *>(b.relu_codes.ptr);
        b.relu_codes_valid = conv_uses_relu_codes(cfg, p, conv_splitk_factor(cfg, p));
        if (!b.relu_codes_valid) p.in_codes = nullptr;
    }
    if (pool) {
        Blob &pt = e->blobs[pool->top_blob];
        p.pool_out = pt.data.f();
        p.pool_mode = pool->pool_mode;
        pt.codes_valid = false;
        pt.amax_data = -1;
        if (conv_fuses_pool(cfg, p)) {
            *pooled = true;
            pt.amax_data = t.amax_data;
            if (conv_writes_pool_codes(cfg) && e->pool_codes) {
                STX_TRY(pt.codes.ensure(pt.count() + 4));
                p.pool_codes = static_cast<unsigned char *>(pt.codes.ptr);
                pt.codes_valid = true;
                p.skip_y = plan.top_unobserved;
            }
        } else {
            p.pool_out = nullptr;
        }
    }
    t.relu_codes_valid = false;
    if (plan.relu_codes && t.relu && plan.conv_reader && conv_h2_enabled()) {
        const size_t bytes = (size_t)t.channels * ((t.h + 1) / 2) * ((t.w + 1) / 2);
        STX_TRY(t.relu_codes.ensure(bytes));
        p.out_codes = static_cast<unsigned char *>(t.relu_codes.ptr);
        t.relu_codes_valid = conv_writes_out_codes(cfg, p, conv_splitk_factor(cfg, p));
        if (!t.relu_codes_valid) p.out_codes = nullptr;
    }
    ProfScope scope(e, "fwd " + L.name, direct);
    return launch_conv(e, cfg, p);
}

static ConvProblem conv_backward_shape(stx_engine *e, int li) {
    const Layer &L = e->layers[li];
    const Blob &b = e->blobs[L.bottom_blob];
    const ConvParams &cp = e->sh->conv[li];
    return conv_bwd_problem(nullptr, nullptr, nullptr, cp.cout, cp.cin, b.h, b.w, cp.ks);
}

static bool conv_backward_takes_pooled(stx_engine *e, int li) {
    const char *env = sw_env("STX_POOL_BWD_FUSE");
    if (env && atoi(env) == 0) return false;
    const ConvProblem p = conv_backward_shape(e, li);
    ConvConfig cfg;
    return p.ksize == 3 && p.M > 4 && conv_choose(p, e->winograd, nullptr, &cfg) == STX_OK &&
           conv_takes_pooled_input(cfg, p);
}

static int run_conv_backward(stx_engine *e, int li, const ConvInject *inj, bool *fused, const Layer *pooled) {
    const Layer &L = e->layers[li];
    Blob &b = e->blobs[L.bottom_blob];
    const Blob &t = e->blobs[L.top_blob];
    const ConvParams &cp = e->sh->conv[li];
    ConvProblem p = conv_backward_shape(e, li);
    p.x = t.diff.f();
    p.y = b.diff.f();
    p.mask = b.relu ? b.data.f() : nullptr;
    p.mask_codes = b.relu && b.relu_codes_valid ? static_cast<const unsigned char *>(b.relu_codes.ptr) : nullptr;
    p.wants_codes = b.relu && b.relu_codes_wanted;
    if (cp.ks == 3 && cp.cin <= 4) {
        if (fused) *fused = false;
        const float *packed = nullptr;
        STX_TRY(get_bank(e, li, conv_small_bank(cp.cout, cp.cin), &packed));
        const double direct = conv_flops(cp.cout, cp.cin, b.h, b.w, cp.ks);
        ProfScope scope(e, "bwd " + L.name, direct);
        e->flop_algorithmic += direct;
        e->flop_issued += direct * 4.0 / p.M;
        return conv_small_launch(e->stream, p.x, packed, p.y, p.mask, p.K, p.M, p.H, p.W);
    }
    ConvConfig cfg;
    STX_TRY(choose_conv(e, li, 1, p, &cfg));
    const bool can_fuse = inj && conv_takes_inject(cfg);
    if (fused) *fused = can_fuse;
    if (can_fuse) p.inject = *inj;
    b.amax_diff = -1;
    if (pooled) {
        const Blob &pt = e->blobs[pooled->top_blob];
        if (!conv_takes_pooled_input(cfg, p) || !pt.codes_valid) {
            set_error("run_conv_backward: %s cannot take the gradient of %s pooled", L.name.c_str(), pt.name.c_str());
            return STX_ERR_UNSUPPORTED;
        }
        p.x = pt.diff.f();
        p.pin_codes = static_cast<const unsigned char *>(pt.codes.ptr);
        p.pin_mode = pooled->pool_mode;
        p.pin_mask = t.relu;
        STX_TRY(amax_for(e, pooled->top_blob, true, &p.x_amax));
    } else if (conv_reads_x_amax(cfg)) {
        STX_TRY(amax_for(e, L.top_blob, true, &p.x_amax));
    }
    if (conv_leaves_y_amax(cfg)) {
        p.y_amax = e->amax_slots(L.bottom_blob, true);
        b.amax_diff = L.bottom_blob;
    }
    STX_TRY(get_packed(e, li, 1, cfg, &p.w));
    STX_TRY(attach_splitk(e, cfg, p));
    ProfScope scope(e, "bwd " + L.name, conv_flops(cp.cout, cp.cin, b.h, b.w, cp.ks));
    return launch_conv(e, cfg, p);
}

static size_t style_term_scratch_floats(int C, int HW) {
    return 2 * (size_t)ceil_div(C * C, 64) + (size_t)symm_num_workgroups(C, HW) + 64;
}

int launch_style_terms(stx_engine *e, hipStream_t stream, const float *feat, int C, int h, int w,
                       const float *target, float *sgrad, float *sc, const std::string &name,
                       const unsigned *f_amax, float *term_scratch, std::vector<SumJob> *defer) {
    const int HW = h * w;
    const bool fused = e->first_gram_valid && e->first_gram_blob >= 0 &&
                       feat == e->blobs[e->first_gram_blob].data.f() && C == 64;
    GramPlan plan = gram_plan(C, HW);
    if (fused) {
        plan.splits = e->first_gram_parts;
        plan.tiles = 1;
        plan.parts = 1;
        plan.partial_floats = (size_t)plan.splits * 64 * 64;
    }
    const int fin_blocks = gram_finish_blocks(plan);
    float *const partials = fused ? e->first_gram.f() : nullptr;
    if (!fused) STX_TRY(e->gram_partials.ensure((plan.partial_floats + 2 * fin_blocks) * sizeof(float)));
    STX_TRY(e->dsym.ensure((size_t)C * C * sizeof(float)));
    const bool gram_h2 = !fused && gram_h2_usable(feat, C, HW);
    const bool symm_h2 = symm_h2_usable(feat, sgrad, C, HW);
    const bool bf3 = !symm_h2 && symm_bf3_usable(feat, sgrad, C, HW);
    if ((gram_h2 || symm_h2) && !f_amax) {
        unsigned *scratch;
        STX_TRY(amax_scratch(e, &scratch));
        ProfScope scope(e, "absmax " + name, 0.0, stream);
        STX_TRY(absmax_launch(stream, feat, (size_t)C * HW, scratch));
        f_amax = scratch;
    }
    if (bf3) STX_TRY(e->dsym_pieces.ensure(symm_pieces_elems(C) * sizeof(unsigned short)));
    unsigned short *pieces = bf3 && C % 64 == 0 ? static_cast<unsigned short *>(e->dsym_pieces.ptr) : nullptr;
    {
        ProfScope scope(e, "gram " + name, 2.0 * C * C * (double)HW, stream);
        if (!fused) STX_TRY(gram_partials_launch(stream, feat, plan, e->gram_partials.f(), gram_h2 ? f_amax : nullptr));
        STX_TRY(gram_finish_launch(stream, fused ? partials : e->gram_partials.f(), plan, nullptr, target,
                                   e->dsym.f(), nullptr, pieces, gram_h2 ? f_amax : nullptr,
                                   defer ? term_scratch : nullptr));
    }
    ProfScope scope(e, "symm " + name, 2.0 * C * C * (double)HW, stream);
    const float *block_sumsq = defer ? term_scratch : (fused ? partials : e->gram_partials.f()) + plan.partial_floats;
    auto finish = [&](float *symm_partials, int n_wg) -> int {
        if (!defer) return sum_partials2_launch(stream, block_sumsq, fin_blocks, sc, symm_partials, n_wg, sc + 1);
        defer->push_back(SumJob{block_sumsq, fin_blocks, sc});
        defer->push_back(SumJob{symm_partials, n_wg, sc + 1});
        return STX_OK;
    };
    if (symm_h2 || bf3) {
        const int n_wg = symm_num_workgroups(C, HW);
        float *symm_partials = defer ? term_scratch + 2 * fin_blocks : nullptr;
        if (!defer) {
            STX_TRY(e->symm_partials.ensure((size_t)n_wg * sizeof(float)));
            symm_partials = e->symm_partials.f();
        }
        if (symm_h2)
            STX_TRY(symm_h2_launch(stream, feat, e->dsym.f(), reinterpret_cast<const unsigned *>(block_sumsq + fin_blocks),
                                   fin_blocks, f_amax, sgrad, symm_partials, C, HW));
        else
            STX_TRY(symm_bf3_launch(stream, feat, e->dsym.f(), static_cast<unsigned short *>(e->dsym_pieces.ptr),
                                    pieces != nullptr, sgrad, symm_partials, C, HW));
        return finish(symm_partials, n_wg);
    }
    const ConvConfig cfg = conv_pick_config(1, C, C, h, w);
    const int n_wg = conv_num_workgroups(cfg, C, h, w);
    STX_TRY(e->symm_partials.ensure((size_t)n_wg * sizeof(float)));
    ConvProblem p{};
    p.x = feat;
    p.w = e->dsym.f();
    p.y = sgrad;
    p.partials = e->symm_partials.f();
    p.K = C;
    p.M = C;
    p.H = h;
    p.W = w;
    p.ksize = 1;
    p.epilogue = kEpiSymm;
    STX_TRY(conv_launch(stream, cfg, p, false));
    return sum_partials2_launch(stream, block_sumsq, fin_blocks, sc, e->symm_partials.f(), n_wg, sc + 1);
}

int launch_masked_style_terms(stx_engine *e, hipStream_t stream, const float *feat, int C, int h, int w,
                              const float *mask_map, const ContentWindow &win, const float *target,
                              float *sgrad, float *sc, const std::string &name, const unsigned *f_amax,
                              float *term_scratch, float *mask_scratch, std::vector<SumJob> *defer) {
    STX_TRY(e->masked_feat.ensure((size_t)C * h * w * sizeof(float)));
    STX_TRY(e->masked_target.ensure((size_t)C * C * sizeof(float)));
    float *const m2_partials = mask_scratch, *const ms_partials = mask_scratch + kMaskParts;
    {
        ProfScope scope(e, "mask " + name, 0.0, stream);
        int n_m2 = 0;
        STX_TRY(mask_apply_launch(stream, feat, mask_map, win, e->masked_feat.f(), m2_partials, &n_m2));
        STX_TRY(mask_target_launch(stream, target, C, m2_partials, n_m2, h * w, e->masked_target.f(), sc + 3));
    }
    STX_TRY(launch_style_terms(e, stream, e->masked_feat.f(), C, h, w, e->masked_target.f(), sgrad, sc, name,
                               f_amax, term_scratch, defer));
    ProfScope scope(e, "smask " + name, 0.0, stream);
    int n_ms = 0;
    STX_TRY(mask_sgrad_launch(stream, sgrad, mask_map, win, sc + 3, ms_partials, &n_ms));
    if (!defer) return sum_partials_launch(stream, ms_partials, n_ms, sc + 2);
    defer->push_back(SumJob{ms_partials, n_ms, sc + 2});
    return STX_OK;
}

int launch_stat_terms(stx_engine *e, hipStream_t stream, const float *feat, int C, int h, int w, const float *MU,
                      const float *SD, float *sgrad, float *sc, const std::string &name, float *stat_scratch,
                      std::vector<SumJob> *defer) {
    const int HW = h * w;
    float *const partials = stat_scratch;
    float *const table = partials + 4 * (size_t)C * stat_slices(HW);
    float *const abs_partials = table + 4 * (size_t)C;
    ProfScope scope(e, "stat " + name, 0.0, stream);
    STX_TRY(stat_partials_launch(stream, feat, C, HW, partials));
    STX_TRY(stat_finish_launch(stream, partials, C, HW, MU, SD, table, sc, nullptr, nullptr));
    int n_parts = 0;
    STX_TRY(stat_grad_launch(stream, feat, C, HW, table, sgrad, abs_partials, &n_parts));
    if (!defer) return sum_partials_launch(stream, abs_partials, n_parts, sc + 1);
    defer->push_back(SumJob{abs_partials, n_parts, sc + 1});
    return STX_OK;
}

static int begin_timing(stx_engine *e) {
    e->ev_cur = (e->ev_cur + 1) % stx_engine::kTimed;
    STX_HIP(hipEventRecord(e->ev_start[e->ev_cur], e->stream));
    e->flop_algorithmic = e->flop_issued = 0;
    return STX_OK;
}

static int end_timing(stx_engine *e) {
    STX_HIP(hipEventRecord(e->ev_stop[e->ev_cur], e->stream));
    if (e->ev_recorded < stx_engine::kTimed) ++e->ev_recorded;
    e->timed = true;
    return STX_OK;
}

namespace {

struct Tap {
    int blob;
    const stx_tap *t;
};

struct TileCall {
    const float *img;
    int img_mem, th, tw, rx, ry, start[2];
    const stx_tap *taps;
    int n_taps;
    float *grad_out;
    int grad_mem;
};

struct TilePlan {
    std::vector<Tap> order;
    std::vector<char> needed;
    std::vector<int> tap_of;
    std::deque<stx_tap> extra;
};

struct Term {
    bool style;
    const float *src;
    const float *sums;
    float coef;
    ContentWindow win;
};

struct TileRun {
    stx_engine *e;
    const TileCall &c;
    const TilePlan &plan;
    PendingLoss &pl;
    bool sums_late;
    bool interleave;
    std::vector<std::vector<Term>> terms;
    std::vector<SumJob> sum_jobs;
    size_t scratch_used;
    std::vector<SumJob> *defer() { return sums_late ? &sum_jobs : nullptr; }
};

}

static const StatTarget *stat_target_of(const stx_engine *e, int blob) {
    for (const StatTarget &t : e->sh->stats)
        if (t.blob == blob) return &t;
    return nullptr;
}

static int sc_grad_prepare(stx_engine *e, const TileCall &c, TilePlan &plan) {
    std::vector<Tap> &order = plan.order;
    const stx_tap *taps = c.taps;
    const int n_taps = c.n_taps;
    for (int i = 0; i < n_taps; ++i) {
        const int blob = e->find_blob(taps[i].layer);
        if (blob <= 0) {
            set_error("stx_sc_grad_tile: unknown tap layer '%s'",
                      taps[i].layer ? taps[i].layer : "(null)");
            return STX_ERR_ARG;
        }
        for (const Tap &o : order)
            if (o.blob == blob) {
                set_error("stx_sc_grad_tile: layer '%s' is tapped twice", taps[i].layer);
                return STX_ERR_ARG;
            }
        if (!taps[i].is_content && !taps[i].is_style && !taps[i].is_dd && !stat_target_of(e, blob)) continue;
        order.push_back(Tap{blob, &taps[i]});
    }
    for (const StatTarget &st : e->sh->stats) {
        bool tapped = false;
        for (const Tap &o : order) tapped |= o.blob == st.blob;
        if (tapped) continue;
        stx_tap t{};
        t.layer_weight = 1.0;
        plan.extra.push_back(t);
        order.push_back(Tap{st.blob, &plan.extra.back()});
    }
    if (order.empty()) {
        set_error("stx_sc_grad_tile: no content, style or Deep-Dream layer");
        return STX_ERR_ARG;
    }
    std::sort(order.begin(), order.end(), [](const Tap &a, const Tap &b) { return a.blob > b.blob; });
    std::vector<char> &needed = plan.needed;
    needed.assign(e->blobs.size(), 0);
    mark_ancestors(e, order[0].blob, needed);
    std::vector<int> &tap_of = plan.tap_of;
    tap_of.assign(e->blobs.size(), -1);
    for (size_t i = 0; i < order.size(); ++i) {
        if (!needed[order[i].blob]) {
            set_error("stx_sc_grad_tile: tapped layers must lie on one path through the network "
                      "('%s' does not feed '%s')", e->blobs[order[i].blob].name.c_str(),
                      e->blobs[order[0].blob].name.c_str());
            return STX_ERR_UNSUPPORTED;
        }
        tap_of[order[i].blob] = (int)i;
    }
    for (const Tap &tp : order) {
        if (tp.t->is_content && e->sh->n_contents == 0) {
            set_error("stx_sc_grad_tile: no content targets set");
            return STX_ERR_STATE;
        }
        if (tp.t->is_style && e->sh->n_styles == 0) {
            set_error("stx_sc_grad_tile: no style targets set");
            return STX_ERR_STATE;
        }
    }

    return shape_blobs(e, c.th, c.tw, needed, true);
}

static ContentWindow content_window(const Blob &b, int ch, int cw, const int start[2], int rx, int ry) {
    ContentWindow win;
    win.C = b.channels;
    win.fh = b.h;
    win.fw = b.w;
    win.ch = ch;
    win.cw = cw;
    win.oy = (int)std::floor((double)start[0] / b.scale);
    win.ox = (int)std::floor((double)start[1] / b.scale);
    win.sx = (int)std::floor((double)rx / b.scale);
    win.sy = (int)std::floor((double)ry / b.scale);
    return win;
}

static ContentWindow dream_window(const Blob &b) {
    const int origin[2] = {0, 0};
    return content_window(b, b.h, b.w, origin, 0, 0);
}

static int queue_residual_term(TileRun &run, size_t k, const char *label, const float *target,
                               const ContentWindow &win, double weight) {
    stx_engine *e = run.e;
    const Blob &b = e->blobs[run.plan.order[k].blob];
    size_t si;
    STX_TRY(alloc_scalars(e, 2 + 2 * 1024, &si));
    float *sums = e->A().scalars.f() + si;
    {
        ProfScope scope(e, label + b.name, 0.0, e->stream);
        STX_TRY(content_sums_launch(e->stream, b.data.f(), target, win, sums, run.defer()));
    }
    run.pl.terms.push_back(LossTerm{si, weight * 0.5});
    run.terms[k].push_back(Term{false, target, sums, (float)weight, win});
    return STX_OK;
}

static int queue_content_terms(TileRun &run, size_t k) {
    stx_engine *e = run.e;
    const Tap &tp = run.plan.order[k];
    const Blob &b = e->blobs[tp.blob];
    bool any = false;
    for (const ContentTarget &ct : e->sh->contents) {
        if (ct.blob != tp.blob) continue;
        any = true;
        const ContentWindow win = content_window(b, ct.h, ct.w, run.c.start, run.c.rx, run.c.ry);
        if (win.oy + win.fh > win.ch || win.ox + win.fw > win.cw) {
            set_error("content window [%d+%d, %d+%d] exceeds the %dx%d map of layer %s",
                      win.oy, win.fh, win.ox, win.fw, win.ch, win.cw, b.name.c_str());
            return STX_ERR_ARG;
        }
        STX_TRY(queue_residual_term(run, k, "content ", ct.feat->f(), win, tp.t->layer_weight * tp.t->content_weight));
    }
    if (!any) {
        set_error("no content target for layer %s", b.name.c_str());
        return STX_ERR_STATE;
// ... 173 lines not shown
    ProfScope scope(e, "inject " + b.name, 0.0);
    b.amax_diff = -1;
    for (size_t ti = 0; ti < terms.size(); ++ti) {
        const Term &t = terms[ti];
        unsigned *amax = nullptr;
        if (ti + 1 == terms.size() && conv_h2_enabled()) {
            amax = e->amax_slots(blob, true);
            b.amax_diff = blob;
        }
        if (t.style)
            STX_TRY(inject_style_launch(e->stream, b.diff.f(), t.src, b.count(), t.sums, t.coef,
                                        diff_written, amax));
        else
            STX_TRY(inject_content_launch(e->stream, b.diff.f(), b.data.f(), t.src, t.win,
                                          t.sums, t.coef, diff_written, amax));
        diff_written = true;
    }
    return STX_OK;
}

static bool tap_fusable(const TileRun &run, size_t k) {
    int ns = 0, nc = 0;
    for (const Term &t : run.terms[k]) {
        if (!t.style && !t.src) return false;
        (t.style ? ns : nc)++;
    }
    return ns <= 1 && nc <= 1;
}

static ConvInject make_inject(const TileRun &run, size_t k, const Blob &bot) {
    ConvInject inj{};
    for (const Term &t : run.terms[k]) {
        if (t.style) {
            inj.sgrad = t.src;
            inj.s_abs_sum = t.sums;
            inj.s_coef = t.coef;
        } else {
            inj.content = t.src;
            inj.c_sums = t.sums;
            inj.c_coef = t.coef;
            inj.win = t.win;
            inj.feat = bot.data.f();
        }
    }
    return inj;
}

static int backward_walk(TileRun &run) {
    stx_engine *e = run.e;
    const int data_blob = e->layers[0].top_blob;
    int cur = run.plan.order[0].blob;
    for (Blob &b : e->blobs) b.amax_diff = -1;
    {
        bool written = false;
        STX_TRY(inject_terms(run, 0, written));
        if (!written)
            STX_HIP(hipMemsetAsync(e->blobs[cur].diff.ptr, 0, e->blobs[cur].count() * sizeof(float),
                                   e->stream));
    }
    const Layer *pooled = nullptr;
    while (cur != data_blob) {
        const int li = e->blobs[cur].producer;
        const Layer &L = e->layers[li];
        Blob &bot = e->blobs[L.bottom_blob];
        const Blob &top = e->blobs[cur];
        const int k = run.plan.tap_of[L.bottom_blob];
        bool fused = false;
        if (L.type == STX_LAYER_POOL && top.codes_valid && k < 0 && L.ksize == 2 && L.stride == 2 && L.pad == 0 &&
            e->layers[bot.producer].type == STX_LAYER_CONV && conv_backward_takes_pooled(e, bot.producer)) {
            pooled = &L;
            cur = L.bottom_blob;
            continue;
        }
        if (L.type == STX_LAYER_CONV) {
            ConvInject inj{};
            if (k >= 0 && tap_fusable(run, (size_t)k)) {
                inj = make_inject(run, (size_t)k, bot);
                fused = true;
            }
            STX_TRY(run_conv_backward(e, li, fused ? &inj : nullptr, &fused, pooled));
            pooled = nullptr;
        } else {
            ProfScope scope(e, "bwd " + L.name, 0.0);
            if (top.codes_valid)
                STX_TRY(pool_backward_codes_launch(
                    e->stream, top.diff.f(), static_cast<const unsigned char *>(top.codes.ptr),
                    bot.channels, bot.h, bot.w, L.pool_mode, bot.relu, bot.diff.f()));
            else
                STX_TRY(pool_backward_launch(e->stream, top.diff.f(), bot.data.f(), bot.channels,
                                             bot.h, bot.w, L.pool_mode, bot.relu, bot.diff.f()));
            bot.amax_diff = top.amax_diff;
        }
        cur = L.bottom_blob;
        if (k >= 0 && !fused) {
            bool written = true;
            STX_HIP(hipMemsetAsync(e->amax_slots(L.bottom_blob, true), 0, kAmaxSlots * sizeof(unsigned), e->stream));
            STX_TRY(inject_terms(run, (size_t)k, written));
        }
    }
    return STX_OK;
}

static void first_gram_setup(stx_engine *e, const TilePlan &plan) {
    const int data_blob = e->layers[0].top_blob;
    e->first_gram_blob = -1;
    e->first_gram_valid = false;
    for (const Tap &tp : plan.order) {
        const int pl = e->blobs[tp.blob].producer;
        bool unmasked = e->sh->masks.empty();
        for (const StyleTarget &st : e->sh->styles)
            unmasked |= st.blob == tp.blob && !style_mask_of(e, st.index, tp.blob);
        if (tp.t->is_style && unmasked && pl > 0 && e->layers[pl].type == STX_LAYER_CONV &&
            e->layers[pl].bottom_blob == data_blob && e->blobs[tp.blob].channels == 64)
            e->first_gram_blob = tp.blob;
    }
}

static int sc_grad_run(stx_engine *e, const TileCall &c, const TilePlan &plan, PendingLoss &pl) {
    const std::vector<Tap> &order = plan.order;
    TileRun run{e, c, plan, pl, !(sw_env("STX_SUMS_LATE") && !atoi(sw_env("STX_SUMS_LATE"))),
                !(sw_env("STX_TERMS_LATE") && atoi(sw_env("STX_TERMS_LATE"))),
                std::vector<std::vector<Term>>(order.size()), {}, 0};
    while (e->sgrad_tap.size() < order.size()) e->sgrad_tap.emplace_back(new DevBuf);
    if (!e->sh->stats.empty())
        while (e->sgrad_stat.size() < order.size()) e->sgrad_stat.emplace_back(new DevBuf);
    {
        size_t need = 0;
        for (const Tap &tp : order) {
            const Blob &b = e->blobs[tp.blob];
            if (stat_target_of(e, tp.blob)) need += stat_scratch_floats(b.channels, b.h * b.w);
            if (!tp.t->is_style) continue;
            for (const StyleTarget &st : e->sh->styles) {
                if (st.blob != tp.blob) continue;
                if (run.sums_late) need += style_term_scratch_floats(b.channels, b.h * b.w);
                if (style_mask_of(e, st.index, tp.blob)) need += kMaskScratchFloats;
            }
        }
        STX_TRY(e->term_scratch.ensure(need * sizeof(float)));
    }
    STX_TRY(begin_timing(e));
    std::vector<char> observed(e->blobs.size(), 0);
    for (const Tap &tp : order) observed[tp.blob] = 1;
    first_gram_setup(e, plan);
    STX_TRY(forward(e, plan.needed, order[0].blob, run.interleave ? &run : nullptr, true, observed));
    if (!run.interleave) {
        for (size_t k = order.size(); k-- > 0;) STX_TRY(queue_tap_terms(run, k));
    }
    if (!run.sum_jobs.empty()) {
        ProfScope scope(e, "sums", 0.0);
        STX_TRY(sum_jobs_launch(e->stream, run.sum_jobs.data(), (int)run.sum_jobs.size()));
    }
    STX_TRY(backward_walk(run));
    STX_TRY(end_timing(e));
    STX_HIP(hipMemcpyAsync(e->A().host, e->A().scalars.ptr, e->A().used * sizeof(float),
                           hipMemcpyDeviceToHost, e->stream));
    return STX_OK;
}

static int sc_grad_eager(stx_engine *e, const TileCall &c, double *loss_out) {
    {
        const size_t per_call = ((size_t)c.n_taps + e->sh->stats.size()) * 2100 *
                                (size_t)std::max(1, e->sh->n_contents + e->sh->n_styles);
        if (e->A().used + per_call > e->scalars_cap) STX_TRY(do_sync(e));
        if (per_call > e->scalars_cap) {
            set_error("stx_sc_grad_tile: %d taps need more scalar space than the arena holds", c.n_taps);
            return STX_ERR_NOMEM;
        }
    }
    TilePlan plan;
    STX_TRY(sc_grad_prepare(e, c, plan));
    Blob &in = e->blobs[e->layers[0].top_blob];
    if (c.img != in.data.ptr) STX_TRY(copy_in(e, in.data.ptr, c.img, c.img_mem, in.count() * sizeof(float)));
    PendingLoss pl;
    pl.out = loss_out;
    STX_TRY(sc_grad_run(e, c, plan, pl));
    if (c.grad_out != in.diff.ptr)
        STX_TRY(copy_out(e, c.grad_out, c.grad_mem, in.diff.ptr, in.count() * sizeof(float)));
    e->A().pending.push_back(std::move(pl));
    ++e->n_tile_evals;
    return STX_OK;
}

}

extern "C" {

int stx_features_tile(stx_engine *e, const float *img, int img_mem, int th, int tw,
                      const char *const *layers, int n_layers, float *const *out, int out_mem) {
    if (!e || !img || th <= 0 || tw <= 0 || n_layers <= 0 || !layers || !out) {
        set_error("stx_features_tile: bad arguments");
        return STX_ERR_ARG;
    }
    STX_TRY(e->set_device());
    std::vector<char> needed(e->blobs.size(), 0);
    std::vector<int> want(n_layers);
    for (int i = 0; i < n_layers; ++i) {
        want[i] = e->find_blob(layers[i]);
        if (want[i] < 0 || !out[i]) {
            set_error("stx_features_tile: unknown layer '%s'", layers[i] ? layers[i] : "(null)");
            return STX_ERR_ARG;
        }
        mark_ancestors(e, want[i], needed);
    }
    STX_TRY(shape_blobs(e, th, tw, needed, false));
    Blob &in = e->blobs[e->layers[0].top_blob];
    STX_TRY(copy_in(e, in.data.ptr, img, img_mem, in.count() * sizeof(float)));
    STX_TRY(begin_timing(e));
    e->first_gram_blob = -1;
    e->first_gram_valid = false;
    const int last_blob = (int)e->blobs.size() - 1;
    std::vector<char> observed(e->blobs.size(), 0);
    for (int i = 0; i < n_layers; ++i) observed[want[i]] = 1;
    STX_TRY(forward(e, needed, needed[last_blob] ? last_blob : -1, nullptr, false, observed));
    STX_TRY(end_timing(e));
    for (int i = 0; i < n_layers; ++i) {
        const Blob &b = e->blobs[want[i]];
        STX_TRY(copy_out(e, out[i], out_mem, b.data.ptr, b.count() * sizeof(float)));
    }
    return STX_OK;
}

int stx_sc_grad_tile(stx_engine *e, const float *img, int img_mem, int th, int tw,
                     const int roll_xy[2], const int start_yx[2], const stx_tap *taps, int n_taps,
                     double *loss_out, float *grad_out, int grad_mem, int sync_now) {
    if (!e || !img || th <= 0 || tw <= 0 || n_taps < 0 || (!taps && n_taps > 0) || !grad_out || !start_yx) {
        set_error("stx_sc_grad_tile: bad arguments");
        return STX_ERR_ARG;
    }
    STX_TRY(e->set_device());
    const TileCall c{img, img_mem, th, tw, roll_xy ? roll_xy[0] : 0, roll_xy ? roll_xy[1] : 0,
                     {start_yx[0], start_yx[1]}, taps, n_taps, grad_out, grad_mem};
    STX_TRY(sc_grad_eager(e, c, loss_out));
    if (sync_now) return do_sync(e);
    return STX_OK;
}

int stx_tile_buffers(stx_engine *e, int th, int tw, float **tile_in, float **grad_out) {
    if (!e || th <= 0 || tw <= 0 || !tile_in || !grad_out) return STX_ERR_ARG;
    STX_TRY(e->set_device());
    Blob &in = e->blobs[e->layers[0].top_blob];
    const size_t bytes = (size_t)in.channels * th * tw * sizeof(float);
    STX_TRY(in.data.ensure(bytes));
    STX_TRY(in.diff.ensure(bytes));
    *tile_in = in.data.f();
    *grad_out = in.diff.f();
    return STX_OK;
}

int stx_gram_matrix(stx_engine *e, const float *feat, int feat_mem, int channels, int hw,
                    float *gram_out, int gram_mem) {
    if (!e || !feat || !gram_out || channels <= 0 || hw <= 0) return STX_ERR_ARG;
    STX_TRY(e->set_device());
    const float *src = feat;
    if (feat_mem == STX_HOST) {
        STX_TRY(e->upload.ensure((size_t)channels * hw * sizeof(float)));
        STX_TRY(copy_in(e, e->upload.ptr, feat, STX_HOST, (size_t)channels * hw * sizeof(float)));
        src = e->upload.f();
    }
    const GramPlan plan = gram_plan(channels, hw);
    STX_TRY(e->gram_partials.ensure(plan.partial_floats * sizeof(float)));
    STX_TRY(e->gram.ensure((size_t)channels * channels * sizeof(float)));
    const unsigned *f_amax = nullptr;
    if (gram_h2_usable(src, channels, hw)) {
        unsigned *scratch;
        STX_TRY(amax_scratch(e, &scratch));
        STX_TRY(absmax_launch(e->stream, src, (size_t)channels * hw, scratch));
        f_amax = scratch;
    }
    STX_TRY(gram_partials_launch(e->stream, src, plan, e->gram_partials.f(), f_amax));
    STX_TRY(gram_finish_launch(e->stream, e->gram_partials.f(), plan, e->gram.f(), nullptr, nullptr,
                               nullptr, nullptr, f_amax));
    STX_TRY(copy_out(e, gram_out, gram_mem, e->gram.ptr, (size_t)channels * channels * sizeof(float)));
    if (feat_mem == STX_HOST || gram_mem == STX_HOST) STX_HIP(hipStreamSynchronize(e->stream));
    return STX_OK;
}

int stx_feature_stats(stx_engine *e, const float *feat, int feat_mem, int channels, int hw, float *mean_out,
                      float *sd_out, int out_mem) {
    if (!e || !feat || !mean_out || !sd_out || channels <= 0 || hw <= 0) return STX_ERR_ARG;
    STX_TRY(e->set_device());
    const float *src = feat;
    if (feat_mem == STX_HOST) {
        STX_TRY(e->upload.ensure((size_t)channels * hw * sizeof(float)));
        STX_TRY(copy_in(e, e->upload.ptr, feat, STX_HOST, (size_t)channels * hw * sizeof(float)));
        src = e->upload.f();
    }
    const size_t parts = 4 * (size_t)channels * stat_slices(hw);
    STX_TRY(e->stat_scratch.ensure((parts + 2 * (size_t)channels) * sizeof(float)));
    float *mu = e->stat_scratch.f() + parts, *sd = mu + channels;
    STX_TRY(stat_partials_launch(e->stream, src, channels, hw, e->stat_scratch.f()));
    STX_TRY(stat_finish_launch(e->stream, e->stat_scratch.f(), channels, hw, nullptr, nullptr, nullptr, nullptr, mu, sd));
    STX_TRY(copy_out(e, mean_out, out_mem, mu, (size_t)channels * sizeof(float)));
    STX_TRY(copy_out(e, sd_out, out_mem, sd, (size_t)channels * sizeof(float)));
    if (feat_mem == STX_HOST || out_mem == STX_HOST) STX_HIP(hipStreamSynchronize(e->stream));
    return STX_OK;
}

}
```

style_transfer_amd/engine.py:

```python

import ctypes

import numpy as np

from . import lib
from .netspec import NetSpec

_TYPE_CODES = {'Input': lib.LAYER_INPUT, 'Convolution': lib.LAYER_CONV, 'ReLU': lib.LAYER_RELU,
               'Pooling': lib.LAYER_POOL}


class DeviceArray:

    def __init__(self, engine, shape, dtype=np.float32):
        self.engine = engine
        self.shape = tuple(int(s) for s in shape)
        self.dtype = np.dtype(dtype)
        self.nbytes = int(np.prod(self.shape, dtype=np.int64)) * self.dtype.itemsize
        ptr = ctypes.c_void_p()
        lib.call('stx_malloc', engine.handle, self.nbytes, ctypes.byref(ptr))
        self.ptr = ptr.value

    @classmethod
    def from_pointer(cls, engine, ptr, shape, dtype=np.float32, owner=None):
# ... 192 lines not shown
        lib.call('stx_set_conv_weights', self.handle, conv_layer.encode(), wp, bp, wmem)
        if wmem == lib.DEVICE:
            self.sync()
        del wkeep, bkeep

    def set_contents_and_styles(self, contents, styles):
        keep = []
        n_c = sum(len(c) for c in contents)
        n_s = sum(len(s) for s in styles)
        ctargets = (lib.ContentTarget * max(1, n_c))()
        starget = (lib.StyleTarget * max(1, n_s))()
        i = 0
        for ci, content in enumerate(contents):
            for layer, feat in content.items():
                ptr, mem, obj = _as_arg(feat)
                keep.append(obj)
                t = ctargets[i]
                t.content_index, t.layer = ci, self._cstr(layer)
                t.channels, t.height, t.width = obj.shape
                t.features, t.mem = ptr, mem
                i += 1
        i = 0
        for si, style in enumerate(styles):
            for layer, gram in style.items():
                ptr, mem, obj = _as_arg(gram)
                keep.append(obj)
                t = starget[i]
                t.style_index, t.layer, t.channels = si, self._cstr(layer), obj.shape[0]
                t.gram, t.mem = ptr, mem
                i += 1
        lib.call('stx_set_contents_and_styles', self.handle, ctargets, n_c, starget, n_s)
        self.n_styles = len(styles)
        self.primary.stat_layers = []

    def set_stat_targets(self, targets, weights=None):
        keep, n = [], len(targets)
        table = (lib.StatTarget * max(1, n))()
        for t, (layer, (mean, sd)) in zip(table, targets.items()):
            mp, mmem, mobj = _as_arg(mean)
            sp, smem, sobj = _as_arg(sd)
            if mmem != smem or mobj.shape != sobj.shape or len(mobj.shape) != 1:
                raise ValueError('statistics target %s: mean and sd are two [C] arrays on the same side' % layer)
            keep += [mobj, sobj]
            t.layer, t.channels, t.mean, t.sd, t.mem = self._cstr(layer), int(mobj.shape[0]), mp, sp, mmem
            t.weight = float(weights.get(layer, 1.0)) if weights is not None else 1.0
        lib.call('stx_set_stat_targets', self.handle, table, n)
        self.primary.stat_layers = list(targets)
        del keep

    def feature_stats(self, feat):
        ptr, mem, keep = _as_arg(feat)
        c = keep.shape[0]
        hw = int(np.prod(keep.shape[1:]))
        mean, sd = np.empty(c, np.float32), np.empty(c, np.float32)
        lib.call('stx_feature_stats', self.handle, ptr, mem, c, hw, mean.ctypes.data, sd.ctypes.data, lib.HOST)
        return mean, sd

    def set_style_masks(self, masks):
        keep, entries = [], []
        for si, mask in enumerate(masks):
            if mask is None:
                continue
            ptr, mem, obj = _as_arg(mask)
            if len(obj.shape) != 2:
                raise ValueError('style mask %d: an [H, W] array is expected, not %s' % (si, tuple(obj.shape)))
            keep.append(obj)
            entries.append((si, int(obj.shape[0]), int(obj.shape[1]), ptr, mem))
        table = (lib.StyleMask * max(1, len(entries)))()
        for t, (si, h, w, ptr, mem) in zip(table, entries):
            t.style_index, t.H, t.W, t.mask, t.mem = si, h, w, ptr, mem
        lib.call('stx_set_style_masks', self.handle, table, len(entries))
        del keep

    def features_tile(self, img, layers):
        ptr, mem, keep = _as_arg(img)
        th, tw = keep.shape[-2:]
        outs = [np.empty(self.feature_shape(l, th, tw), np.float32) for l in layers]
        names = (ctypes.c_char_p * len(layers))(*[l.encode() for l in layers])
        ptrs = (ctypes.c_void_p * len(layers))(*[o.ctypes.data for o in outs])
        lib.call('stx_features_tile', self.handle, ptr, mem, th, tw, names, len(layers), ptrs,
                 lib.HOST)
        self.sync()
        return dict(zip(layers, outs))

    def features_tile_device(self, img, layers, out=None):
        ptr, mem, keep = _as_arg(img)
        th, tw = keep.shape[-2:]
        if out is None:
            out = {}
        for l in layers:
            shape = self.feature_shape(l, th, tw)
            if l not in out or out[l].shape != shape:
                out[l] = self.empty(shape)
        names = (ctypes.c_char_p * len(layers))(*[l.encode() for l in layers])
        ptrs = (ctypes.c_void_p * len(layers))(*[out[l].ptr for l in layers])
        lib.call('stx_features_tile', self.handle, ptr, mem, th, tw, names, len(layers), ptrs,
                 lib.DEVICE)
        if mem == lib.HOST:
            self.sync()
        return out

    def map_place(self, dst, y0, x0, src):
        c, h, w = src.shape
        lib.call('stx_map_place', self.handle, dst.ptr, c, dst.shape[1], dst.shape[2], int(y0),
                 int(x0), src.ptr, h, w)

    def map_roll_add(self, acc, src, roll_xy, alpha, init_divisor=0.0):
        c, h, w = src.shape
        roll = (ctypes.c_int * 2)(int(roll_xy[0]), int(roll_xy[1]))
        lib.call('stx_map_roll_add', self.handle, acc.ptr, src.ptr, c, h, w, roll, float(alpha),
                 float(init_divisor))

    def _taps(self, content_layers, style_layers, layer_weights, content_weight, style_weight,
              dd_layers=(), dd_weight=None):
        names = list(dict.fromkeys(list(content_layers) + list(style_layers) + list(dd_layers) +
                                   list(self.primary.stat_layers)))
        taps = (lib.Tap * len(names))()
        for t, name in zip(taps, names):
            t.layer = self._cstr(name)
            t.layer_weight = float(layer_weights.get(name, 1.0)) if layer_weights else 1.0
            t.is_content = int(name in content_layers)
            t.content_weight = float(content_weight.get(name, 0.0)) if t.is_content else 0.0
            t.is_style = int(name in style_layers)
            t.style_weight = float(style_weight.get(name, 0.0)) if t.is_style else 0.0
            t.is_dd = int(name in dd_layers)
            t.dd_weight = float(dd_weight.get(name, 0.0)) if t.is_dd and dd_weight else 0.0
        return taps, len(names)

    def io_buffers(self, th, tw):
        tin, gout = ctypes.c_void_p(), ctypes.c_void_p()
        lib.call('stx_tile_buffers', self.handle, int(th), int(tw), ctypes.byref(tin), ctypes.byref(gout))
        return (DeviceArray.from_pointer(self, tin.value, (3, th, tw)),
                DeviceArray.from_pointer(self, gout.value, (3, th, tw)))

    def sc_grad_tile_async(self, img, start, roll, content_layers, style_layers, layer_weights,
                           content_weight, style_weight, grad_out=None, dd_layers=(),
                           dd_weight=None):
        ptr, mem, keep = _as_arg(img)
        th, tw = keep.shape[-2:]
        if grad_out is None:
            grad_out = np.empty((3, th, tw), np.float32)
        gptr, gmem, gkeep = (grad_out.ptr, lib.DEVICE, grad_out) \
            if isinstance(grad_out, DeviceArray) else (grad_out.ctypes.data, lib.HOST, grad_out)
        taps, n_taps = self._taps(content_layers, style_layers, layer_weights, content_weight,
                                  style_weight, dd_layers, dd_weight)
        roll_c = (ctypes.c_int * 2)(int(roll[0]), int(roll[1])) if roll is not None \
            else (ctypes.c_int * 2)(0, 0)
        start_c = (ctypes.c_int * 2)(int(start[0]), int(start[1]))
        pending = self.keep_until_sync(PendingTile(gkeep, (keep, taps)))
        lib.call('stx_sc_grad_tile', self.handle, ptr, mem, th, tw, roll_c, start_c, taps, n_taps,
                 ctypes.byref(pending._loss), gptr, gmem, 0)
        return pending

    def sc_grad_tile(self, img, start, roll, content_layers, style_layers, layer_weights,
                     content_weight, style_weight, dd_layers=(), dd_weight=None):
        pending = self.sc_grad_tile_async(img, start, roll, content_layers, style_layers,
                                          layer_weights, content_weight, style_weight,
                                          dd_layers=dd_layers, dd_weight=dd_weight)
        self.sync()
        return pending.loss, pending.grad

    def gram_matrix(self, feat):
        ptr, mem, keep = _as_arg(feat)
        c = keep.shape[0]
        hw = int(np.prod(keep.shape[1:]))
        out = np.empty((c, c), np.float32)
        lib.call('stx_gram_matrix', self.handle, ptr, mem, c, hw, out.ctypes.data, lib.HOST)
        return out

    def profile(self, on=True):
        lib.call('stx_profile_enable', self.handle, int(on))

    def profile_read(self, clock=False):
        buf = ctypes.create_string_buffer(1 << 20)
        lib.call('stx_profile_read', self.handle, buf, len(buf), None)
        rows = []
        for line in buf.value.decode().splitlines():
            label, ms, flops, mhz = line.split('\t')
            rows.append((label, float(ms), float(flops), float(mhz)) if clock else
                        (label, float(ms), float(flops)))
        return rows

    def last_tile_flops(self):
        a, b = ctypes.c_double(0), ctypes.c_double(0)
        lib.call('stx_last_tile_flops', self.handle, ctypes.byref(a), ctypes.byref(b))
        return a.value, b.value

    def clock_marks(self, on):
        lib.call('stx_clock_marks', self.handle, 1 if on else 0)

    def clock_marks_read(self, max_values=16384):
        mhz = (ctypes.c_double * max_values)()
        n = ctypes.c_int(0)
        lib.call('stx_clock_marks_read', self.handle, mhz, max_values, ctypes.byref(n))
        return [mhz[i] for i in range(n.value)]

    def last_tile_ms(self):
        ms = ctypes.c_float(0)
        lib.call('stx_last_tile_ms', self.handle, ctypes.byref(ms))
        return ms.value
```

style_transfer_amd/farm.py:

```python

import os

import numpy as np

from . import image_ops
from .engine import DeviceArray, TileEngine


def tile_grid(img_hw, tile_size):
    h, w = int(img_hw[0]), int(img_hw[1])
    ny, nx = (h - 1) // tile_size + 1, (w - 1) // tile_size + 1
    th, tw = h // ny, w // nx
    rects = []
    for y in range(ny):
        for x in range(nx):
            y0, x0 = y * th, x * tw
            rects.append((y0, h if y == ny - 1 else y0 + th, x0, w if x == nx - 1 else x0 + tw))
    return rects


class LazyLoss:

    def __init__(self):
        self.parts, self.engines, self._value, self._tickets = [], [], None, None

    def add(self, part, engine):
        assert self._value is None
        self.parts.append(part)
        if engine not in self.engines:
            self.engines.append(engine)
        return self

    def seal(self, also=()):
        assert self._value is None and self._tickets is None
        for eng in also:
            if eng not in self.engines:
                self.engines.append(eng)
        self._tickets = [(eng, eng.fence()) for eng in self.engines]
        return self

    def __float__(self):
        if self._value is None:
            if self._tickets is not None:
                for eng, ticket in self._tickets:
                    eng.wait_fence(ticket)
            else:
                for eng in self.engines:
                    eng.sync()
            self._value = float(sum(p.loss if hasattr(p, 'loss') else p.value for p in self.parts))
            self.parts, self.engines, self._tickets = [], [], None
        return self._value


class TileFarm:

    def __init__(self, net, devices=(0,), weights=None, verbose=True, engines=None,
                 streams_per_device=None, force_staging=None):
        if streams_per_device is None:
            streams_per_device = int(os.environ.get('STX_STREAMS_PER_GPU', '2'))
        self.net = net
        self.verbose = verbose
        self.force_staging = bool(int(os.environ.get('STX_FARM_FORCE_STAGING', '0'))) \
            if force_staging is None else bool(force_staging)
        self.owns_engines = engines is None
        self.zero_copy = not bool(int(os.environ.get('STX_FARM_COPY_TILES', '0')))
        self.devices = list(devices)
        self.weights = weights
        self.max_engines = len(self.devices) * max(1, streams_per_device) \
            if engines is None else len(engines)
        self.engines = engines if engines is not None else []
        if engines is None:
            for d in self.devices:
                self.engines.append(self._new_engine(d))
        self.master = self.engines[0]
        self._targets = None
        self._tiles = {}
        self._staging = {}
        self.tile_evals = 0

    def _new_engine(self, device):
        for eng in self.engines:
            if eng.device == device:
                return TileEngine(self.net, device, share=eng)
        return TileEngine(self.net, device, self.weights)

    def primaries(self):
        out = []
        for eng in self.engines:
            if eng.primary not in out:
                out.append(eng.primary)
        return out

    def close(self):
        for bufs in list(self._tiles.values()) + list(self._staging.values()):
            for b in bufs:
                b.free()
        self._tiles.clear()
        self._staging.clear()
        if self.owns_engines:
            for e in self.engines:
                e.close()

    def layers(self):
        return self.net.blob_names()

    def layer_info(self, layer):
        return self.net.layer_info(layer)

    def set_weights(self, weights):
        self.weights = weights
        for e in self.primaries():
            for name, (w, b) in weights.items():
                e.set_weights(name, w, b)

    def set_contents_and_styles(self, contents, styles):
        self._targets = (contents, styles)
        for e in self.engines:
            e.sync()
        for e in self.primaries():
            e.set_contents_and_styles(contents, styles)

    def set_style_masks(self, masks):
        for e in self.engines:
            e.sync()
        for e in self.primaries():
            e.set_style_masks(masks)

    def set_stat_targets(self, targets, weights=None):
        for e in self.engines:
            e.sync()
        for e in self.primaries():
            e.set_stat_targets(targets, weights)

    def feature_stats(self, feat):
        return self.master.feature_stats(feat)

    def _engines_for(self, n_tiles):
        want = min(self.max_engines, max(len(self.devices), n_tiles))
        while len(self.engines) < want and self.owns_engines:
            self.engines.append(self._new_engine(self.devices[len(self.engines) % len(self.devices)]))
        return self.engines[:want]

    def eval_features_once(self, img, layers, tile_size=512):
        img = np.ascontiguousarray(img, np.float32)
        hw = np.array(img.shape[-2:])
        rects = tile_grid(hw, tile_size)
        if len(rects) > 1 and self.verbose:
            nx = (hw[1] - 1) // tile_size + 1
            print('Using %dx%d tiles of size %dx%d.' %
                  (nx, len(rects) // nx, rects[0][3] - rects[0][2], rects[0][1] - rects[0][0]))
        feats = {}
        for layer in layers:
            scale, ch = self.layer_info(layer)
            feats[layer] = np.zeros((ch,) + tuple(np.int32(np.ceil(hw / scale))), np.float32)
        for t, (y0, y1, x0, x1) in enumerate(rects):
            eng = self.engines[t % len(self.engines)]
            tile_feats = eng.features_tile(img[:, y0:y1, x0:x1], list(layers))
            for layer, f in tile_feats.items():
                scale, _ = self.layer_info(layer)
                fy, fx = y0 // scale, x0 // scale
                feats[layer][:, fy:fy + f.shape[1], fx:fx + f.shape[2]] = f
        return feats

    def prepare_features(self, img, layers, tile_size=512, passes=10):
        img = np.array(img, np.float32)
        hw = np.array(img.shape[-2:])
        if max(hw) <= tile_size:
            passes = 1
        feats = {}
        for i in range(passes):
            xy = np.array((0, 0))
            if i > 0:
                xy = np.int32(np.random.uniform(size=2) * hw) // 32
            self._roll_host(img, xy * 32)
            for layer, f in feats.items():
                self._roll_host(f, xy * 32 // self.layer_info(layer)[0])
            once = self.eval_features_once(img, layers, tile_size)
            for layer in layers:
                if i == 0:
                    feats[layer] = once[layer] / passes
                else:
                    feats[layer] += np.float32(1 / passes) * once[layer]
            self._roll_host(img, -xy * 32)
            for layer, f in feats.items():
                self._roll_host(f, -xy * 32 // self.layer_info(layer)[0])
        return feats

    def prepare_features_device(self, img, layers, tile_size=512, passes=10, roll=None):
        eng = self.master
        on_device = isinstance(img, DeviceArray)
        if on_device:
            assert img.engine is eng and img.dtype == np.float32, 'a float32 picture on the master GPU'
        else:
            img = np.ascontiguousarray(img, np.float32)
        hw = np.array(img.shape[-2:])
        if max(hw) <= tile_size:
            passes = 1
        d_img = img if on_device else eng.to_device(img)
        rects = tile_grid(hw, tile_size)
        if len(rects) > 1 and self.verbose:
            nx = (hw[1] - 1) // tile_size + 1
            print('Using %dx%d tiles of size %dx%d (x %d passes).' %
                  (nx, len(rects) // nx, rects[0][3] - rects[0][2], rects[0][1] - rects[0][0],
                   passes))
        full, acc = {}, {}
        for layer in layers:
            scale, ch = self.layer_info(layer)
            shape = (ch,) + tuple(int(v) for v in np.int32(np.ceil(hw / scale)))
            full[layer] = eng.empty(shape).zero()
            acc[layer] = eng.empty(shape)
        tiles, tile_feats = {}, {}
        for i in range(passes):
            xy = np.array((0, 0))
            if i > 0:
                xy = np.int32(np.random.uniform(size=2) * hw) // 32
            shift = xy * 32
            cut_shift = shift if roll is None else shift + np.asarray(roll, np.int64)
            for rect in rects:
                th, tw = rect[1] - rect[0], rect[3] - rect[2]
                if (th, tw) not in tiles:
                    tiles[(th, tw)] = eng.empty((3, th, tw))
                    tile_feats[(th, tw)] = {}
                tile = tiles[(th, tw)]
                image_ops.cut_tile(eng, d_img, cut_shift, rect, tile)
                feats = eng.features_tile_device(tile, list(layers), tile_feats[(th, tw)])
                for layer in layers:
                    scale, _ = self.layer_info(layer)
                    eng.map_place(full[layer], rect[0] // scale, rect[2] // scale, feats[layer])
            for layer in layers:
                scale, _ = self.layer_info(layer)
                back = -(shift // scale)
                eng.map_roll_add(acc[layer], full[layer], back, 1 / passes,
                                 init_divisor=passes if i == 0 else 0.0)
        eng.sync()
        for bufs in list(tile_feats.values()):
            for b in bufs.values():
                b.free()
        for b in list(tiles.values()) + list(full.values()) + ([] if on_device else [d_img]):
            b.free()
        return acc

    @staticmethod
    def _roll_host(arr, xy):
        if np.any(np.asarray(xy) != 0):
            arr[...] = np.roll(arr, (int(xy[0]), int(xy[1])), axis=(-1, -2))
        return arr

    def gram_matrix(self, feat):
        return self.master.gram_matrix(feat)

    def _tile_buffers(self, ei, slot, th, tw):
        key = (ei, slot, th, tw)
        if key not in self._tiles:
            eng = self.engines[ei]
            self._tiles[key] = (eng.empty((3, th, tw)), eng.empty((3, th, tw)))
        return self._tiles[key]

    def _staging_buffers(self, slot, th, tw):
        key = (slot, th, tw)
        if key not in self._staging:
            self._staging[key] = (self.master.empty((3, th, tw)), self.master.empty((3, th, tw)))
        return self._staging[key]

    def eval_sc_grad(self, img, grad, roll, content_layers, style_layers, layer_weights,
                     content_weight, style_weight, tile_size, dd_layers=(), dd_weight=None,
                     content_roll=None, lazy=False):
        if content_roll is None:
            content_roll = roll
        rects = tile_grid(img.shape[-2:], tile_size)
        engines = self._engines_for(len(rects))
        n = len(engines)
        master = self.master
        jobs, workers = [], []
        one_each = len(rects) <= n and self.zero_copy
        for t, rect in enumerate(rects):
            ei, slot = t % n, t // n
            eng = engines[ei]
            th, tw = rect[1] - rect[0], rect[3] - rect[2]
            if eng.device == master.device and not (self.force_staging and ei != 0):
                tile, tgrad = eng.io_buffers(th, tw) if one_each else self._tile_buffers(ei, slot, th, tw)
            else:
                tile, tgrad = self._staging_buffers(t, th, tw)
            image_ops.cut_tile(master, img, roll, rect, tile)
            if eng is not master and eng not in workers:
                workers.append(eng)
            jobs.append((eng, rect, tile, tgrad))
        for eng in workers:
            eng.wait_for(master)
        loss = LazyLoss()
        for eng, rect, tile, tgrad in jobs:
            loss.add(eng.sc_grad_tile_async(
                tile, (rect[0], rect[2]), content_roll, content_layers, style_layers,
                layer_weights, content_weight, style_weight, grad_out=tgrad,
                dd_layers=dd_layers, dd_weight=dd_weight), eng)
        for eng in workers:
            master.wait_for(eng)
        for eng, rect, tile, tgrad in jobs:
            image_ops.put_tile(master, grad, roll, rect, tgrad)
        self.tile_evals += len(rects)
        if lazy:
            return loss
        value = float(loss)
        master.sync()
        return value
```

style_transfer_amd/lib.py:

```python

import ctypes
import os

_HERE = os.path.dirname(os.path.abspath(__file__))
LIB_PATH = os.environ.get('STX_LIB') or os.path.join(_HERE, 'csrc', 'libstx.so')

HOST, DEVICE = 0, 1
LAYER_INPUT, LAYER_CONV, LAYER_RELU, LAYER_POOL = 0, 1, 2, 3
POOL_MAX, POOL_AVE = 0, 1
(Q_SHARED_ENGINES, Q_TARGET_UPLOADS, Q_TARGET_BYTES, Q_WEIGHT_BYTES, Q_TILE_EVALS,
 Q_PEERS_WITHOUT_ACCESS) = range(6)

c_float_p = ctypes.POINTER(ctypes.c_float)
c_double_p = ctypes.POINTER(ctypes.c_double)
c_int_p = ctypes.POINTER(ctypes.c_int)


class StxError(RuntimeError):

    def __init__(self, func, code, message):
        super().__init__('%s failed with status %d: %s' % (func, code, message))
        self.code = code


class LayerDesc(ctypes.Structure):
    _fields_ = [('name', ctypes.c_char_p), ('type', ctypes.c_int), ('bottom', ctypes.c_char_p),
                ('top', ctypes.c_char_p), ('num_output', ctypes.c_int),
                ('kernel_size', ctypes.c_int), ('pad', ctypes.c_int), ('stride', ctypes.c_int),
                ('pool_mode', ctypes.c_int)]


class ContentTarget(ctypes.Structure):
    _fields_ = [('content_index', ctypes.c_int), ('layer', ctypes.c_char_p),
                ('channels', ctypes.c_int), ('height', ctypes.c_int), ('width', ctypes.c_int),
                ('features', ctypes.c_void_p), ('mem', ctypes.c_int)]


class StyleTarget(ctypes.Structure):
    _fields_ = [('style_index', ctypes.c_int), ('layer', ctypes.c_char_p),
                ('channels', ctypes.c_int), ('gram', ctypes.c_void_p), ('mem', ctypes.c_int)]


class StyleMask(ctypes.Structure):
    _fields_ = [('style_index', ctypes.c_int), ('H', ctypes.c_int), ('W', ctypes.c_int),
                ('mask', ctypes.c_void_p), ('mem', ctypes.c_int)]


class StatTarget(ctypes.Structure):
    _fields_ = [('layer', ctypes.c_char_p), ('channels', ctypes.c_int), ('mean', ctypes.c_void_p),
                ('sd', ctypes.c_void_p), ('mem', ctypes.c_int), ('weight', ctypes.c_double)]


class Tap(ctypes.Structure):
    _fields_ = [('layer', ctypes.c_char_p), ('layer_weight', ctypes.c_double),
                ('is_content', ctypes.c_int), ('content_weight', ctypes.c_double),
                ('is_style', ctypes.c_int), ('style_weight', ctypes.c_double),
                ('is_dd', ctypes.c_int), ('dd_weight', ctypes.c_double)]


_vp, _i, _sz, _d = ctypes.c_void_p, ctypes.c_int, ctypes.c_size_t, ctypes.c_double
SIGNATURES = {
    'stx_reread_env': [],
    'stx_device_count': [c_int_p],
    'stx_device_name': [_i, ctypes.c_char_p, _sz],
    'stx_engine_create': [_i, ctypes.POINTER(LayerDesc), _i, ctypes.POINTER(_vp)],
    'stx_engine_create_shared': [_vp, ctypes.POINTER(_vp)],
    'stx_engine_wait': [_vp, _vp],
    'stx_engine_query': [_vp, _i, c_double_p],
    'stx_set_conv_weights': [_vp, ctypes.c_char_p, _vp, _vp, _i],
    'stx_sync': [_vp],
    'stx_fence': [_vp, ctypes.POINTER(ctypes.c_ulonglong)],
    'stx_fence_wait': [_vp, ctypes.c_ulonglong],
    'stx_engine_device': [_vp, c_int_p],
    'stx_engine_stream': [_vp, ctypes.POINTER(_vp)],
    'stx_malloc': [_vp, _sz, ctypes.POINTER(_vp)],
    'stx_free': [_vp, _vp],
    'stx_memset_async': [_vp, _vp, _i, _sz],
    'stx_memcpy_async': [_vp, _vp, _i, _vp, _i, _sz],
    'stx_set_contents_and_styles': [_vp, ctypes.POINTER(ContentTarget), _i,
                                    ctypes.POINTER(StyleTarget), _i],
    'stx_set_style_masks': [_vp, ctypes.POINTER(StyleMask), _i],
    'stx_set_stat_targets': [_vp, ctypes.POINTER(StatTarget), _i],
    'stx_features_tile': [_vp, _vp, _i, _i, _i, ctypes.POINTER(ctypes.c_char_p), _i,
                          ctypes.POINTER(_vp), _i],
    'stx_sc_grad_tile': [_vp, _vp, _i, _i, _i, c_int_p, c_int_p, ctypes.POINTER(Tap), _i,
                         c_double_p, _vp, _i, _i],
    'stx_tile_buffers': [_vp, _i, _i, ctypes.POINTER(_vp), ctypes.POINTER(_vp)],
    'stx_gram_matrix': [_vp, _vp, _i, _i, _i, _vp, _i],
    'stx_feature_stats': [_vp, _vp, _i, _i, _i, _vp, _vp, _i],
    'stx_image_cut_tile': [_vp, _vp, _i, _i, c_int_p, _i, _i, _i, _i, _vp],
    'stx_image_put_tile': [_vp, _vp, _i, _i, c_int_p, _i, _i, _i, _i, _vp],
    'stx_image_mask_map': [_vp, _vp, _i, _i, _i, _vp],
    'stx_map_place': [_vp, _vp, _i, _i, _i, _i, _i, _vp, _i, _i],
    'stx_map_roll_add': [_vp, _vp, _vp, _i, _i, _i, c_int_p, _d, _d],
    'stx_image_resample': [_vp, _vp, _i, _i, _i, _vp, _i, _i, c_int_p, c_double_p, _i, c_int_p,
                           c_double_p, _i, _i],
    'stx_image_regularizers': [_vp, _vp, _vp, _i, _i, c_float_p, _d, _d, _d, _d, _vp, _d,
                               c_int_p, c_double_p],
    'stx_image_swt_haar': [_vp, _vp, _vp, _i, _i, c_int_p, _d, _d, c_double_p],
    'stx_image_swt_haar_levels': [_vp, _vp, _vp, _i, _i, _i, c_int_p, _d, _d, c_double_p],
    'stx_image_swt_daub_levels': [_vp, _vp, _vp, _i, _i, _i, _i, c_int_p, _d, _d, c_double_p],
    'stx_image_lap_target': [_vp, _vp, _i, _i, _i, c_int_p, _vp],
    'stx_image_lap': [_vp, _vp, _vp, _i, _i, _i, c_int_p, c_double_p, _vp, _d, c_double_p],
    'stx_adam_step': [_vp, _vp, _vp, _vp, _vp, _vp, _vp, _sz, _d, _d, _d, _d, _d, _d, _d],
    'stx_vec_dot': [_vp, _vp, _vp, _sz, c_double_p],
    'stx_vec_axpy': [_vp, _d, _vp, _vp, _sz],
    'stx_vec_scale': [_vp, _d, _vp, _sz],
    'stx_vec_mean_abs': [_vp, _vp, _sz, c_double_p],
    'stx_vec_dot_async': [_vp, _vp, _vp, _sz, _vp],
    'stx_vec_abs_sum_async': [_vp, _vp, _sz, _vp],
    'stx_vec_axpy_dev': [_vp, _d, _vp, _d, _d, _vp, _d, _vp, _vp, _sz],
    'stx_vec_scale_dev': [_vp, _d, _vp, _d, _vp, _sz],
    'stx_vec_axpy_dot_dev': [_vp, _d, _vp, _d, _d, _vp, _d, _d, _vp, _d, _vp, _vp, _vp, _vp, _sz, _vp],
    'stx_vec_lbfgs_pair': [_vp, _vp, _vp, _vp, _vp, _sz, _vp, c_double_p],
    'stx_vec_scale2_axpy': [_vp, _d, _d, _vp, _vp, _sz],
    'stx_image_step_stats': [_vp, _vp, _vp, _i, _i, c_double_p],
    'stx_image_step_stats_async': [_vp, _vp, _vp, _i, _i, c_double_p],
    'stx_image_to_u8': [_vp, _vp, _i, _i, c_float_p, _vp],
    'stx_image_to_u8_luma': [_vp, _vp, _vp, _i, _i, c_float_p, _vp],
    'stx_image_color_stats': [_vp, _vp, _i, _i, c_double_p],
    'stx_image_color_affine': [_vp, _vp, _vp, _i, _i, c_double_p, c_double_p, c_float_p],
    'stx_op_conv_forward': [_vp, _vp, _i, _i, _i, _vp, _vp, _i, _i, _i, _vp],
    'stx_op_conv_backward_data': [_vp, _vp, _i, _i, _i, _vp, _i, _i, _vp, _vp],
    'stx_op_pool_forward': [_vp, _vp, _i, _i, _i, _i, _vp],
    'stx_op_pool_backward': [_vp, _vp, _vp, _i, _i, _i, _i, _vp, _vp],
    'stx_op_style_terms': [_vp, _vp, _i, _i, _i, _vp, _vp, _vp, c_double_p, c_double_p],
    'stx_op_masked_style_terms': [_vp, _vp, _i, _i, _i, _vp, _i, _i, _i, _i, c_int_p, _vp, _vp, c_double_p],
    'stx_op_stat_terms': [_vp, _vp, _i, _i, _i, _vp, _vp, _vp, c_double_p],
    'stx_op_content_terms': [_vp, _vp, _i, _i, _i, _vp, _i, _i, _i, _i, c_int_p, _vp, c_double_p],
    'stx_last_tile_ms': [_vp, c_float_p],
    'stx_last_tile_flops': [_vp, c_double_p, c_double_p],
    'stx_clock_marks': [_vp, ctypes.c_int],
    'stx_clock_marks_read': [_vp, c_double_p, ctypes.c_int, ctypes.POINTER(ctypes.c_int)],
    'stx_profile_enable': [_vp, _i],
    'stx_profile_read': [_vp, ctypes.c_char_p, _sz, ctypes.POINTER(_sz)],
}
NON_STATUS = {'stx_version': (ctypes.c_char_p, []), 'stx_last_error': (ctypes.c_char_p, []),
              'stx_engine_destroy': (None, [_vp]),
              'stx_image_lap_floats': (_sz, [_i, _i, _i, c_int_p])}

_lib = None


def load():
    global _lib
    if _lib is not None:
        return _lib
    if not os.path.exists(LIB_PATH):
        raise ImportError('%s is missing: build the HIP extension first '
                          '(python -m style_transfer_amd.build)' % LIB_PATH)
    lib = ctypes.CDLL(LIB_PATH, mode=ctypes.RTLD_GLOBAL)
    for name, argtypes in SIGNATURES.items():
        fn = getattr(lib, name)
        fn.argtypes, fn.restype = argtypes, ctypes.c_int
    for name, (restype, argtypes) in NON_STATUS.items():
        fn = getattr(lib, name)
        fn.argtypes, fn.restype = argtypes, restype
    _lib = lib
    return lib


def call(name, *args):
    lib = load()
    rc = getattr(lib, name)(*args)
    if rc != 0:
        raise StxError(name, rc, lib.stx_last_error().decode('utf-8', 'replace'))


def reread_env():
    if _lib is not None:
        call('stx_reread_env')


def device_count():
    n = ctypes.c_int(0)
    call('stx_device_count', ctypes.byref(n))
    return n.value


def device_name(device):
    buf = ctypes.create_string_buffer(256)
    call('stx_device_name', device, buf, 256)
    return buf.value.decode()


def version():
    return load().stx_version().decode()
```

Measured before the change: 273.1.

## Read tile input and write tile gradient directly from the full image window

```diff
diff --git a/include/stx.h b/include/stx.h
--- a/include/stx.h
+++ b/include/stx.h
@@ -129,6 +129,11 @@
 
 int stx_tile_buffers(stx_engine *e, int th, int tw, float **tile_in, float **grad_out);
 
+int stx_sc_grad_window(stx_engine *e, const float *img, float *grad, int H, int W, const int image_roll_xy[2],
+                       int y0, int x0, int th, int tw, const int roll_xy[2], const int start_yx[2],
+                       const stx_tap *taps, int n_taps, double *loss_out, int sync_now);
+int stx_tile_window_enabled(int *enabled);
+
 int stx_gram_matrix(stx_engine *e, const float *feat, int feat_mem, int channels, int hw,
                     float *gram_out, int gram_mem);
 
diff --git a/style_transfer_amd/csrc/common.h b/style_transfer_amd/csrc/common.h
--- a/style_transfer_amd/csrc/common.h
+++ b/style_transfer_amd/csrc/common.h
@@ -216,8 +216,11 @@
 
 bool conv_first_usable(int K, int M, int ksize);
 int conv_first_workgroups(int H, int W);
+struct ImageWindow { int H, W, sy0, sx0; };
+bool conv_first_window_usable(int K, int H, int W, const ImageWindow &win);
 int conv_first_launch(hipStream_t s, const float *x, const float *w_caffe, const float *bias, float *y,
-                      int K, int H, int W, int relu, float *gram_partials, unsigned *y_amax = nullptr);
+                      int K, int H, int W, int relu, float *gram_partials, unsigned *y_amax = nullptr,
+                      const ImageWindow *win = nullptr);
 
 ConvConfig wino2_config(int geometry = 0);
 int wino2_pick_geometry(int H, int W);
@@ -249,7 +252,7 @@
 int conv_small_pack(hipStream_t s, const float *w_caffe, int Mo, int Ko, int transpose_flip,
                     float *packed);
 int conv_small_launch(hipStream_t s, const float *x, const float *packed, float *y,
-                      const float *mask, int K, int M, int H, int W);
+                      const float *mask, int K, int M, int H, int W, const ImageWindow *win = nullptr);
 
 bool conv_h2_enabled();
 struct ConvTuner { int device; hipStream_t stream; hipEvent_t ev0, ev1; std::function<int(const ConvConfig &, const float **)> bank; };
diff --git a/style_transfer_amd/csrc/conv_first.hip b/style_transfer_amd/csrc/conv_first.hip
--- a/style_transfer_amd/csrc/conv_first.hip
+++ b/style_transfer_amd/csrc/conv_first.hip
@@ -33,11 +33,12 @@
     float *gram;
     unsigned *y_amax;
     int K, H, W, tiles_x, n_tiles, relu, vec_store, strided;
+    int sH, sW, sy0, sx0;
 };
 
 }
 
-template <bool GRAM, int STORE>
+template <bool GRAM, int STORE, bool WIN>
 __global__ __launch_bounds__(kNT, GRAM ? 2 : 3) void conv_first_kernel(FirstArgs a) {
     constexpr int kWork = 2 * kPatch + kTile;
     static_assert(kFM * kFM <= kWork, "the Gram tile must fit the working set");
@@ -65,7 +66,7 @@
     asm volatile("" ::"v"(bias_r[0]), "v"(bias_r[1]));
 
     const __amdgpu_buffer_rsrc_t rx = __builtin_amdgcn_make_buffer_rsrc(
-        const_cast<float *>(a.x), 0, (int)((size_t)a.K * HW * 4), 0x00020000);
+        const_cast<float *>(a.x), 0, (int)((size_t)a.K * (WIN ? (size_t)a.sH * a.sW : HW) * 4), 0x00020000);
     constexpr unsigned kOob = 0x80000000u;
     int p_row[kPL], p_col[kPL], p_off[kPL];
 #pragma unroll
@@ -76,7 +77,7 @@
         const bool live = e < 9 * (kFP + 2) && c < a.K;
         p_row[n] = live ? r - 1 : -(1 << 28);
         p_col[n] = col - 1;
-        p_off[n] = (c * a.H + r - 1) * a.W + col - 1;
+        p_off[n] = WIN ? c * a.sH * a.sW : (c * a.H + r - 1) * a.W + col - 1;
     }
     auto patch_load = [&](int t, float (&preg)[kPL]) {
         const int ty = sgpr(t < 0 ? -4 : t / a.tiles_x);
@@ -85,7 +86,15 @@
 #pragma unroll
         for (int n = 0; n < kPL; ++n) {
             const bool ok = (unsigned)(ty + p_row[n]) < (unsigned)a.H && (unsigned)(x0 + p_col[n]) < (unsigned)a.W;
-            const unsigned off = ok ? (unsigned)(origin + p_off[n]) * 4u : kOob;
+            unsigned off;
+            if (WIN) {
+                int sr = a.sy0 + ty + p_row[n], sc = a.sx0 + x0 + p_col[n];
+                sr = sr >= a.sH ? sr - a.sH : sr;
+                sc = sc >= a.sW ? sc - a.sW : sc;
+                off = ok ? (unsigned)(p_off[n] + sr * a.sW + sc) * 4u : kOob;
+            } else {
+                off = ok ? (unsigned)(origin + p_off[n]) * 4u : kOob;
+            }
             preg[n] = __builtin_bit_cast(float, __builtin_amdgcn_raw_buffer_load_b32(rx, off, 0, 0));
         }
     };
@@ -275,8 +284,19 @@
     return (int)std::min<long>(tiles, env ? atoi(env) : 768);
 }
 
+bool conv_first_window_usable(int K, int H, int W, const ImageWindow &win) {
+    return win.H >= H && win.W >= W && win.sy0 >= 0 && win.sy0 < win.H && win.sx0 >= 0 && win.sx0 < win.W &&
+           4.0 * K * (double)win.H * win.W < 2147483648.0;
+}
+
 int conv_first_launch(hipStream_t s, const float *x, const float *w_caffe, const float *bias, float *y,
-                      int K, int H, int W, int relu, float *gram_partials, unsigned *y_amax) {
+                      int K, int H, int W, int relu, float *gram_partials, unsigned *y_amax,
+                      const ImageWindow *win) {
+    if (win && !conv_first_window_usable(K, H, W, *win)) {
+        set_error("conv_first_launch: a %d x %d window of a %d x %d picture cannot be read in place", H, W,
+                  win->H, win->W);
+        return STX_ERR_UNSUPPORTED;
+    }
     if (4.0 * K * (double)H * W >= 2147483648.0) {
         set_error("conv_first_launch: a %d x %d plane is beyond the buffer-addressing limit", H, W);
         return STX_ERR_UNSUPPORTED;
@@ -295,13 +315,21 @@
     a.n_tiles = H * a.tiles_x;
     a.relu = relu;
     a.vec_store = W % 4 == 0 && (reinterpret_cast<uintptr_t>(y) & 15) == 0;
+    a.sH = win ? win->H : H;
+    a.sW = win ? win->W : W;
+    a.sy0 = win ? win->sy0 : 0;
+    a.sx0 = win ? win->sx0 : 0;
     const int grid = gram_partials ? conv_first_workgroups(H, W) : conv_first_plain_workgroups(H, W);
     {
         const char *env = sw_env("STX_FIRST_STRIDED");
         a.strided = env && atoi(env) != 0;
     }
     const int store = 4.0 * kFM * (double)H * W >= 4294967280.0 ? 2 : a.vec_store ? 0 : 1;
-#define STX_FIRST(G, S) conv_first_kernel<G, S><<<grid, kNT, 0, s>>>(a)
+#define STX_FIRST(G, S)                                                \
+    do {                                                               \
+        if (win) conv_first_kernel<G, S, true><<<grid, kNT, 0, s>>>(a); \
+        else conv_first_kernel<G, S, false><<<grid, kNT, 0, s>>>(a);    \
+    } while (0)
     if (gram_partials) {
         if (store == 0) STX_FIRST(true, 0);
         else if (store == 1) STX_FIRST(true, 1);
diff --git a/style_transfer_amd/csrc/conv_mfma.hip b/style_transfer_amd/csrc/conv_mfma.hip
--- a/style_transfer_amd/csrc/conv_mfma.hip
+++ b/style_transfer_amd/csrc/conv_mfma.hip
@@ -698,6 +698,7 @@
     const float *mask;
     int K, M, H, W, n_chunks, tiles_x, x_bytes, w_bytes;
     int n_wg, wg_per_xcd;
+    int wH, wW, wy0, wx0;
 };
 
 template <int KC, int PR, bool VEC>
@@ -830,17 +831,23 @@
         }
     }
     const int xx = x0 + lane;
+    const bool win = a.wH > 0;
+    const size_t plane = win ? (size_t)a.wH * a.wW : (size_t)HW;
+    int wx = a.wx0 + xx;
+    wx = wx >= a.wW ? wx - a.wW : wx;
 #pragma unroll
     for (int r = 0; r < RW; ++r) {
         const int yy = y0 + wave * RW + r;
         if (yy < a.H && xx < a.W) {
+            int wy = a.wy0 + yy;
+            wy = wy >= a.wH ? wy - a.wH : wy;
+            const size_t dst = win ? (size_t)wy * a.wW + wx : (size_t)yy * a.W + xx;
 #pragma unroll
             for (int m = 0; m < 4; ++m) {
                 if (m < a.M) {
-                    const size_t idx = (size_t)m * HW + (size_t)yy * a.W + xx;
                     float v = acc[r][m];
-                    if (a.mask) v = a.mask[idx] > 0.f ? v : 0.f;
-                    a.y[idx] = v;
+                    if (a.mask) v = a.mask[(size_t)m * HW + (size_t)yy * a.W + xx] > 0.f ? v : 0.f;
+                    a.y[(size_t)m * plane + dst] = v;
                 }
             }
         }
@@ -874,9 +881,14 @@
 }
 
 int conv_small_launch(hipStream_t s, const float *x, const float *packed, float *y,
-                      const float *mask, int K, int M, int H, int W) {
+                      const float *mask, int K, int M, int H, int W, const ImageWindow *win) {
     if (M > 4) {
         set_error("conv_small_launch: M = %d > 4", M);
+        return STX_ERR_ARG;
+    }
+    if (win && !(win->H >= H && win->W >= W && win->sy0 >= 0 && win->sy0 < win->H && win->sx0 >= 0 &&
+                 win->sx0 < win->W)) {
+        set_error("conv_small_launch: a %d x %d window of a %d x %d picture", H, W, win->H, win->W);
         return STX_ERR_ARG;
     }
     const double xb = 4.0 * K * (double)H * W;
@@ -899,6 +911,10 @@
     a.tiles_x = ceil_div(W, 64);
     a.x_bytes = big ? 0 : (int)xb;
     a.w_bytes = (int)(conv_small_packed_floats(K) * 4);
+    a.wH = win ? win->H : 0;
+    a.wW = win ? win->W : 0;
+    a.wy0 = win ? win->sy0 : 0;
+    a.wx0 = win ? win->sx0 : 0;
     const char *novec = sw_env("STX_SMALL_NOVEC");
     const bool vec = W % 4 == 0 && (reinterpret_cast<uintptr_t>(x) & 15) == 0 && !(novec && atoi(novec));
     const bool tall = (long)a.tiles_x * ceil_div(H, kSmallPR) >= 1024;
diff --git a/style_transfer_amd/csrc/engine.cpp b/style_transfer_amd/csrc/engine.cpp
--- a/style_transfer_amd/csrc/engine.cpp
+++ b/style_transfer_amd/csrc/engine.cpp
@@ -66,11 +66,26 @@
     }
     a.pending.clear();
     a.used = 0;
+    a.unmirrored = false;
     a.dused = 0;
     a.ticket = 0;
 }
 
+bool tile_window_enabled() {
+    const char *env = sw_env("STX_TILE_WINDOW");
+    return !(env && atoi(env) == 0);
+}
+
+int mirror_scalars(stx_engine *e) {
+    stx_engine::ScalarArena &a = e->A();
+    if (a.unmirrored && a.used > 0)
+        STX_HIP(hipMemcpyAsync(a.host, a.scalars.ptr, a.used * sizeof(float), hipMemcpyDeviceToHost, e->stream));
+    a.unmirrored = false;
+    return STX_OK;
+}
+
 int do_sync(stx_engine *e) {
+    STX_TRY(mirror_scalars(e));
     STX_HIP(hipStreamSynchronize(e->stream));
     publish_arena(e->arena[e->cur ^ 1]);
     publish_arena(e->arena[e->cur]);
@@ -454,6 +469,7 @@
     if (!e || !ticket) return STX_ERR_ARG;
     STX_TRY(e->set_device());
     stx_engine::ScalarArena &a = e->A();
+    STX_TRY(mirror_scalars(e));
     STX_HIP(hipEventRecord(a.fence, e->stream));
     a.ticket = e->next_ticket++;
     *ticket = a.ticket;
diff --git a/style_transfer_amd/csrc/engine.h b/style_transfer_amd/csrc/engine.h
--- a/style_transfer_amd/csrc/engine.h
+++ b/style_transfer_amd/csrc/engine.h
@@ -146,6 +146,13 @@
     DevBuf first_gram;
     int first_gram_blob = -1, first_gram_parts = 0;
     bool first_gram_valid = false;
+    struct TileWindow {
+        const float *img;
+        float *grad;
+        int rx, ry, y0, x0;
+        ImageWindow map;
+    };
+    const TileWindow *window = nullptr;
     DevBuf gram_partials, gram, dsym, dsym_pieces, symm_partials, upload;
     DevBuf term_scratch;
     DevBuf masked_feat, masked_target;
@@ -154,6 +161,7 @@
         DevBuf scalars;
         float *host = nullptr;
         size_t used = 0;
+        bool unmirrored = false;
         DevBuf dscalars;
         double *dhost = nullptr;
         size_t dused = 0;
@@ -246,6 +254,8 @@
 int copy_in(stx_engine *e, void *dst, const void *src, int mem, size_t bytes);
 int copy_out(stx_engine *e, void *dst, int mem, const void *src, size_t bytes);
 int do_sync(stx_engine *e);
+int mirror_scalars(stx_engine *e);
+bool tile_window_enabled();
 ConvProblem conv_fwd_problem(const float *x, float *y, const float *bias, int Cin, int Cout, int H, int W,
                              int ks, int relu);
 ConvProblem conv_bwd_problem(const float *dy, float *dx, const float *mask, int Cout, int Cin, int H, int W,
diff --git a/style_transfer_amd/csrc/tile_path.cpp b/style_transfer_amd/csrc/tile_path.cpp
--- a/style_transfer_amd/csrc/tile_path.cpp
+++ b/style_transfer_amd/csrc/tile_path.cpp
@@ -173,6 +173,15 @@
     }
     plan.top_unobserved = plan.pool && !observed[L.top_blob] && L.top_blob != relu_blob && readers == 1;
     return plan;
+}
+
+static int window_cut(stx_engine *e, Blob &in) {
+    const stx_engine::TileWindow &w = *e->window;
+    return cut_tile_launch(e->stream, w.img, w.map.H, w.map.W, w.rx, w.ry, w.y0, w.x0, in.h, in.w, in.data.f());
+}
+static int window_put(stx_engine *e, const Blob &in) {
+    const stx_engine::TileWindow &w = *e->window;
+    return put_tile_launch(e->stream, w.grad, w.map.H, w.map.W, w.rx, w.ry, w.y0, w.x0, in.h, in.w, in.diff.f());
 }
 
 static int run_conv_forward(stx_engine *e, int li, const FwdConvPlan &plan, bool *pooled) {
@@ -206,8 +215,14 @@
         ProfScope scope(e, "fwd " + L.name, direct);
         e->flop_algorithmic += direct;
         e->flop_issued += direct;
+        const stx_engine::TileWindow *win = L.bottom_blob == e->layers[0].top_blob ? e->window : nullptr;
+        if (win && conv_first_window_usable(cp.cin, b.h, b.w, win->map))
+            return conv_first_launch(e->stream, win->img, cp.w.f(), cp.b.f(), p.y, cp.cin, b.h, b.w, p.relu, gram,
+                                     y_amax, &win->map);
+        if (win) STX_TRY(window_cut(e, b));
         return conv_first_launch(e->stream, p.x, cp.w.f(), cp.b.f(), p.y, cp.cin, b.h, b.w, p.relu, gram, y_amax);
     }
+    if (e->window && L.bottom_blob == e->layers[0].top_blob) STX_TRY(window_cut(e, b));
     ConvConfig cfg;
     STX_TRY(choose_conv(e, li, 0, p, &cfg));
     b.relu_codes_wanted = !conv_reads_x_amax(cfg) && !b.relu_codes_valid && plan.relu_codes && b.relu && b.channels <= 128;
@@ -293,6 +308,9 @@
         ProfScope scope(e, "bwd " + L.name, direct);
         e->flop_algorithmic += direct;
         e->flop_issued += direct * 4.0 / p.M;
+        if (e->window && L.bottom_blob == e->layers[0].top_blob)
+            return conv_small_launch(e->stream, p.x, packed, e->window->grad, p.mask, p.K, p.M, p.H, p.W,
+                                     &e->window->map);
         return conv_small_launch(e->stream, p.x, packed, p.y, p.mask, p.K, p.M, p.H, p.W);
     }
     ConvConfig cfg;
@@ -322,7 +340,9 @@
     STX_TRY(get_packed(e, li, 1, cfg, &p.w));
     STX_TRY(attach_splitk(e, cfg, p));
     ProfScope scope(e, "bwd " + L.name, conv_flops(cp.cout, cp.cin, b.h, b.w, cp.ks));
-    return launch_conv(e, cfg, p);
+    STX_TRY(launch_conv(e, cfg, p));
+    if (e->window && L.bottom_blob == e->layers[0].top_blob) STX_TRY(window_put(e, b));
+    return STX_OK;
 }
 
 static size_t style_term_scratch_floats(int C, int HW) {
@@ -474,6 +494,7 @@
     int n_taps;
     float *grad_out;
     int grad_mem;
+    const stx_engine::TileWindow *window;
 };
 
 struct TilePlan {
@@ -953,8 +974,8 @@
     }
     STX_TRY(backward_walk(run));
     STX_TRY(end_timing(e));
-    STX_HIP(hipMemcpyAsync(e->A().host, e->A().scalars.ptr, e->A().used * sizeof(float),
-                           hipMemcpyDeviceToHost, e->stream));
+    e->A().unmirrored = true;
+    if (!tile_window_enabled()) STX_TRY(mirror_scalars(e));
     return STX_OK;
 }
 
@@ -971,12 +992,19 @@
     TilePlan plan;
     STX_TRY(sc_grad_prepare(e, c, plan));
     Blob &in = e->blobs[e->layers[0].top_blob];
-    if (c.img != in.data.ptr) STX_TRY(copy_in(e, in.data.ptr, c.img, c.img_mem, in.count() * sizeof(float)));
     PendingLoss pl;
     pl.out = loss_out;
-    STX_TRY(sc_grad_run(e, c, plan, pl));
-    if (c.grad_out != in.diff.ptr)
-        STX_TRY(copy_out(e, c.grad_out, c.grad_mem, in.diff.ptr, in.count() * sizeof(float)));
+    if (c.window) {
+        e->window = c.window;
+        const int rc = sc_grad_run(e, c, plan, pl);
+        e->window = nullptr;
+        STX_TRY(rc);
+    } else {
+        if (c.img != in.data.ptr) STX_TRY(copy_in(e, in.data.ptr, c.img, c.img_mem, in.count() * sizeof(float)));
+        STX_TRY(sc_grad_run(e, c, plan, pl));
+        if (c.grad_out != in.diff.ptr)
+            STX_TRY(copy_out(e, c.grad_out, c.grad_mem, in.diff.ptr, in.count() * sizeof(float)));
+    }
     e->A().pending.push_back(std::move(pl));
     ++e->n_tile_evals;
     return STX_OK;
@@ -1030,9 +1058,40 @@
     }
     STX_TRY(e->set_device());
     const TileCall c{img, img_mem, th, tw, roll_xy ? roll_xy[0] : 0, roll_xy ? roll_xy[1] : 0,
-                     {start_yx[0], start_yx[1]}, taps, n_taps, grad_out, grad_mem};
+                     {start_yx[0], start_yx[1]}, taps, n_taps, grad_out, grad_mem, nullptr};
     STX_TRY(sc_grad_eager(e, c, loss_out));
     if (sync_now) return do_sync(e);
+    return STX_OK;
+}
+
+int stx_sc_grad_window(stx_engine *e, const float *img, float *grad, int H, int W, const int image_roll_xy[2],
+                       int y0, int x0, int th, int tw, const int roll_xy[2], const int start_yx[2],
+                       const stx_tap *taps, int n_taps, double *loss_out, int sync_now) {
+    if (!e || !img || !grad || H <= 0 || W <= 0 || th <= 0 || tw <= 0 || n_taps < 0 || (!taps && n_taps > 0) ||
+        !start_yx) {
+        set_error("stx_sc_grad_window: bad arguments");
+        return STX_ERR_ARG;
+    }
+    if (y0 < 0 || x0 < 0 || th > H - y0 || tw > W - x0) {
+        set_error("stx_sc_grad_window: the tile %d x %d at (%d, %d) is no rectangle of a %d x %d picture", th, tw,
+                  y0, x0, H, W);
+        return STX_ERR_ARG;
+    }
+    STX_TRY(e->set_device());
+    const int irx = image_roll_xy ? image_roll_xy[0] : 0, iry = image_roll_xy ? image_roll_xy[1] : 0;
+    auto wrap = [](long v, int n) { return (int)(((v % n) + n) % n); };
+    const stx_engine::TileWindow win{img, grad, irx, iry, y0, x0,
+                                     ImageWindow{H, W, wrap((long)y0 - iry, H), wrap((long)x0 - irx, W)}};
+    const TileCall c{nullptr, STX_DEVICE, th, tw, roll_xy ? roll_xy[0] : 0, roll_xy ? roll_xy[1] : 0,
+                     {start_yx[0], start_yx[1]}, taps, n_taps, nullptr, STX_DEVICE, &win};
+    STX_TRY(sc_grad_eager(e, c, loss_out));
+    if (sync_now) return do_sync(e);
+    return STX_OK;
+}
+
+int stx_tile_window_enabled(int *enabled) {
+    if (!enabled) return STX_ERR_ARG;
+    *enabled = tile_window_enabled() ? 1 : 0;
     return STX_OK;
 }
 
diff --git a/style_transfer_amd/engine.py b/style_transfer_amd/engine.py
--- a/style_transfer_amd/engine.py
+++ b/style_transfer_amd/engine.py
@@ -368,6 +368,25 @@
                  ctypes.byref(pending._loss), gptr, gmem, 0)
         return pending
 
+    def sc_grad_window_async(self, img, grad, image_roll, rect, roll, content_layers, style_layers,
+                             layer_weights, content_weight, style_weight, dd_layers=(),
+                             dd_weight=None):
+        assert isinstance(img, DeviceArray) and isinstance(grad, DeviceArray)
+        assert img.shape == grad.shape and img.dtype == grad.dtype == np.float32
+        _, H, W = img.shape
+        y0, y1, x0, x1 = (int(v) for v in rect)
+        taps, n_taps = self._taps(content_layers, style_layers, layer_weights, content_weight,
+                                  style_weight, dd_layers, dd_weight)
+        iroll_c = (ctypes.c_int * 2)(int(image_roll[0]), int(image_roll[1])) \
+            if image_roll is not None else (ctypes.c_int * 2)(0, 0)
+        roll_c = (ctypes.c_int * 2)(int(roll[0]), int(roll[1])) if roll is not None \
+            else (ctypes.c_int * 2)(0, 0)
+        start_c = (ctypes.c_int * 2)(y0, x0)
+        pending = self.keep_until_sync(PendingTile(None, (img, grad, taps)))
+        lib.call('stx_sc_grad_window', self.handle, img.ptr, grad.ptr, H, W, iroll_c, y0, x0,
+                 y1 - y0, x1 - x0, roll_c, start_c, taps, n_taps, ctypes.byref(pending._loss), 0)
+        return pending
+
     def sc_grad_tile(self, img, start, roll, content_layers, style_layers, layer_weights,
                      content_weight, style_weight, dd_layers=(), dd_weight=None):
         pending = self.sc_grad_tile_async(img, start, roll, content_layers, style_layers,
diff --git a/style_transfer_amd/farm.py b/style_transfer_amd/farm.py
--- a/style_transfer_amd/farm.py
+++ b/style_transfer_amd/farm.py
@@ -3,7 +3,7 @@
 
 import numpy as np
 
-from . import image_ops
+from . import image_ops, lib
 from .engine import DeviceArray, TileEngine
 
 
@@ -271,17 +271,21 @@
         engines = self._engines_for(len(rects))
         n = len(engines)
         master = self.master
+        window = self.zero_copy and not self.force_staging and lib.tile_window_enabled()
         jobs, workers = [], []
         one_each = len(rects) <= n and self.zero_copy
         for t, rect in enumerate(rects):
             ei, slot = t % n, t // n
             eng = engines[ei]
             th, tw = rect[1] - rect[0], rect[3] - rect[2]
+            tile = tgrad = None
             if eng.device == master.device and not (self.force_staging and ei != 0):
-                tile, tgrad = eng.io_buffers(th, tw) if one_each else self._tile_buffers(ei, slot, th, tw)
+                if not window:
+                    tile, tgrad = eng.io_buffers(th, tw) if one_each else self._tile_buffers(ei, slot, th, tw)
             else:
                 tile, tgrad = self._staging_buffers(t, th, tw)
-            image_ops.cut_tile(master, img, roll, rect, tile)
+            if tile is not None:
+                image_ops.cut_tile(master, img, roll, rect, tile)
             if eng is not master and eng not in workers:
                 workers.append(eng)
             jobs.append((eng, rect, tile, tgrad))
@@ -289,6 +293,12 @@
             eng.wait_for(master)
         loss = LazyLoss()
         for eng, rect, tile, tgrad in jobs:
+            if tile is None:
+                loss.add(eng.sc_grad_window_async(
+                    img, grad, roll, rect, content_roll, content_layers, style_layers,
+                    layer_weights, content_weight, style_weight,
+                    dd_layers=dd_layers, dd_weight=dd_weight), eng)
+                continue
             loss.add(eng.sc_grad_tile_async(
                 tile, (rect[0], rect[2]), content_roll, content_layers, style_layers,
                 layer_weights, content_weight, style_weight, grad_out=tgrad,
@@ -296,7 +306,8 @@
         for eng in workers:
             master.wait_for(eng)
         for eng, rect, tile, tgrad in jobs:
-            image_ops.put_tile(master, grad, roll, rect, tgrad)
+            if tile is not None:
+                image_ops.put_tile(master, grad, roll, rect, tgrad)
         self.tile_evals += len(rects)
         if lazy:
             return loss
diff --git a/style_transfer_amd/lib.py b/style_transfer_amd/lib.py
--- a/style_transfer_amd/lib.py
+++ b/style_transfer_amd/lib.py
@@ -86,6 +86,9 @@
     'stx_sc_grad_tile': [_vp, _vp, _i, _i, _i, c_int_p, c_int_p, ctypes.POINTER(Tap), _i,
                          c_double_p, _vp, _i, _i],
     'stx_tile_buffers': [_vp, _i, _i, ctypes.POINTER(_vp), ctypes.POINTER(_vp)],
+    'stx_sc_grad_window': [_vp, _vp, _vp, _i, _i, c_int_p, _i, _i, _i, _i, c_int_p, c_int_p,
+                           ctypes.POINTER(Tap), _i, c_double_p, _i],
+    'stx_tile_window_enabled': [c_int_p],
     'stx_gram_matrix': [_vp, _vp, _i, _i, _i, _vp, _i],
     'stx_feature_stats': [_vp, _vp, _i, _i, _i, _vp, _vp, _i],
     'stx_image_cut_tile': [_vp, _vp, _i, _i, c_int_p, _i, _i, _i, _i, _vp],
@@ -172,6 +175,12 @@
         call('stx_reread_env')
 
 
+def tile_window_enabled():
+    on = ctypes.c_int(1)
+    call('stx_tile_window_enabled', ctypes.byref(on))
+    return bool(on.value)
+
+
 def device_count():
     n = ctypes.c_int(0)
     call('stx_device_count', ctypes.byref(n))
```

Result: no change. 274.4, median of 5 (+0.5%).
